# gorgonia/agogo

Hardware: AMD Instinct MI355X
Metric: mcts_sims_per_sec (higher is better)
Workload: dtype f32 (Winograd F(5x5,3x3): fp32 transforms; transform-domain products as fp16x2 = each fp32 operand scaled by a power of two and split into 2 fp16 pieces (22-23 significand bits, absolute error <= 2^-38 of the tensor range), 3 fp16 MFMAs per product, fp32 accumulate)

## Files before the change

### agogo_amd/capi.py

```python
import ctypes as C
import os

import numpy as np

_HERE = os.path.dirname(os.path.abspath(__file__))
_LIB = None

NONE, BLACK, WHITE = 0, 1, 2
PASS, RESIGN = -1, -2
NO_MOVE = -32768
GAME_MNK, GAME_C4, GAME_KOMI, GAME_WQ = 0, 1, 2, 3
ENC_TWOPLANE, ENC_WQ = 0, 1
INF_NET, INF_DUMMY, INF_SCRIPT, INF_HASH, INF_UNIFORM, INF_CALLBACK = 0, 1, 2, 3, 4, 5
BN_DEGENERATE_EPS, BN_RUNNING, BN_IDENTITY = 0, 1, 2
COMPUTE_F32_MFMA, COMPUTE_BF16X3, COMPUTE_FP16X2, COMPUTE_WINO, COMPUTE_AUTO, COMPUTE_WINO_H2 = 0, 1, 2, 3, 4, 5
COMPUTE_FORCE = 0x100
PROF_CONV, PROF_HEADS, PROF_SELECT, PROF_EXPAND, PROF_MOVE, PROF_CONV_INIT = 0, 1, 2, 3, 4, 5
PROF_WINO_IN, PROF_WINO_GEMM, PROF_WINO_OUT = 6, 7, 8
DONT_PREFER_PASS, PREFER_PASS, DONT_RESIGN = 0, 1, 2
POOL_STRICT, POOL_STOP_SEARCH, POOL_GROW = 0, 1, 2


class AgzError(RuntimeError):
    pass
# ... 113 lines not shown
    sig("agz_net_set_bn_stats", i32, vp, i32, pf, pf, C.c_size_t)
    sig("agz_net_init_random", i32, vp, u64)
    sig("agz_net_commit", i32, vp)
    sig("agz_net_infer", i32, vp, pf, i32, pf, pf)
    sig("agz_net_infer_dev", i32, vp, vp, i32, vp, vp)
    sig("agz_host_alloc", i32, vp, C.c_size_t, pvp)
    sig("agz_host_free", i32, vp, vp)
    sig("agz_mcts_to_dot", i32, vp, i32, C.c_char_p, C.c_size_t, C.POINTER(C.c_size_t))
    sig("agz_mcts_set_timeout_ms", i32, vp, i32)
    sig("agz_mcts_last_simulations", i32, vp, C.POINTER(C.c_int64))
    sig("agz_net_set_latency_mode", i32, vp, i32)
    sig("agz_net_set_tower_queues", i32, vp, i32)
    sig("agz_net_set_compute_mode", i32, vp, i32)
    sig("agz_net_flops_per_eval", f64, vp)
    sig("agz_net_save", i32, vp, C.c_char_p)
    sig("agz_net_load", i32, vp, C.c_char_p)
    sig("agz_arena_get_results", i32, vp, C.POINTER(C.c_int64), C.POINTER(C.c_int64), C.POINTER(C.c_int64))
    sig("agz_trainer_create", i32, vp, C.POINTER(NetConf), pvp)
    sig("agz_trainer_destroy", None, vp)
    sig("agz_trainer_num_params", i32, vp)
    sig("agz_trainer_param_info", i32, vp, i32, C.c_char_p, C.c_size_t, C.POINTER(C.c_size_t))
    sig("agz_trainer_set_param", i32, vp, i32, pf, C.c_size_t)
    sig("agz_trainer_get_param", i32, vp, i32, pf, C.c_size_t)
    sig("agz_trainer_get_grad", i32, vp, i32, pf, C.c_size_t)
    sig("agz_trainer_init_random", i32, vp, u64)
    sig("agz_trainer_batch", i32, vp, pf, pf, pf, C.c_float, pf)
    sig("agz_trainer_forward_backward", i32, vp, pf, pf, pf, pf)
    sig("agz_trainer_forward_backward_dev", i32, vp, vp, vp, vp, pf)
    sig("agz_trainer_apply", i32, vp, C.c_float, C.c_float)
    sig("agz_trainer_grads_dev", i32, vp, pvp, C.POINTER(C.c_size_t))
    sig("agz_trainer_set_solver", i32, vp, C.POINTER(SolverConf))
    sig("agz_trainer_get_solver", i32, vp, C.POINTER(SolverConf))
    sig("agz_trainer_get_velocity", i32, vp, i32, pf, C.c_size_t)
    sig("agz_trainer_set_velocity", i32, vp, i32, pf, C.c_size_t)
    sig("agz_trainer_reset_solver", i32, vp)
    sig("agz_trainer_set_compute_mode", i32, vp, i32)
    sig("agz_train", i32, vp, pf, pf, pf, i32, i32, u64, pf)
    sig("agz_trainer_export", i32, vp, vp)
    sig("agz_trainer_save", i32, vp, C.c_char_p)
    sig("agz_trainer_load", i32, vp, C.c_char_p)
    sig("agz_arena_create", i32, vp, C.POINTER(GameConf), C.POINTER(MctsConf), i32, u64, i32, pvp)
    sig("agz_arena_destroy", None, vp)
    sig("agz_arena_set_inferencer", i32, vp, i32, i32, vp)
    sig("agz_arena_reset", i32, vp, pu8)
    sig("agz_arena_play", i32, vp, i32, i32)
    sig("agz_arena_selfplay", i32, vp, C.c_int64, i32)
    sig("agz_arena_set_parallel", i32, vp, i32)
    sig("agz_arena_begin_move", i32, vp)
    sig("agz_arena_simulate", i32, vp, i32)
    sig("agz_arena_end_move", i32, vp, i32)
    sig("agz_arena_apply_moves", i32, vp, pi)
    sig("agz_arena_get_stats", i32, vp, C.POINTER(ArenaStats))
    sig("agz_arena_get_game", i32, vp, i32, pi, C.POINTER(GameState))
    sig("agz_arena_get_history", i32, vp, i32, pi, i32, pi)
    sig("agz_arena_root_children", i32, vp, i32, i32, pi, pu, pf, pf, i32, pi)
    sig("agz_arena_tree_nodes", i32, vp, i32, i32, pi)
    sig("agz_arena_get_examples", i32, vp, pf, pf, pf, pi, i32, pi)
    sig("agz_arena_clear_examples", i32, vp)
    sig("agz_arena_drop_labelled_examples", i32, vp)
    sig("agz_arena_examples_dev", i32, vp, pvp, pvp, pvp, pi)
    i64, pi64 = C.c_int64, C.POINTER(C.c_int64)
    sig("agz_train_dev", i32, vp, vp, vp, vp, i32, i32, u64, pf)
    sig("agz_examples_create", i32, vp, i32, i32, i32, i32, pvp)
    sig("agz_examples_destroy", None, vp)
    sig("agz_examples_count", i32, vp, pi64)
    sig("agz_examples_clear", i32, vp)
    sig("agz_examples_append_arena", i32, vp, vp)
    sig("agz_examples_append_dev", i32, vp, vp, vp, vp, i64)
    sig("agz_examples_append_host", i32, vp, pf, pf, pf, i64)
    sig("agz_examples_get", i32, vp, pf, pf, pf, i64, pi64)
    sig("agz_examples_augment_rotate", i32, vp)
    sig("agz_examples_prepare", i32, vp, i32, i32, u64, pi)
    sig("agz_examples_tensors_dev", i32, vp, pvp, pvp, pvp, pi64, pi)
    sig("agz_examples_get_tensors", i32, vp, pf, pf, pf)
    sig("agz_examples_raw_dev", i32, vp, pvp, pvp, pvp)
    sig("agz_rotate_boards", i32, vp, pf, i32, i32, i32, pf)
    sig("agz_ctx_prof_set_stride", i32, vp, i32, i32)
    sig("agz_wino_stages", i32, vp, pf, pf, i32, i32, i32, i32, i32, pf, pf)
    sig("agz_wino_h2_tile", i32, i32, i32)
    sig("agz_net_set_wino_h2_form", i32, vp, i32)
    sig("agz_net_set_wino_h2_gemm", i32, vp, i32)
    sig("agz_net_min_same_batch", i32, vp, i32, i32, C.POINTER(C.c_int))
    sig("agz_arena_set_prep_compact", i32, vp, i32)
    sig("agz_trainer_set_dma_forward", i32, vp, i32)
    sig("agz_arena_last_prep_batch", i32, vp, C.POINTER(C.c_int), C.POINTER(C.c_int))
    sig("agz_arena_debug_counter", i32, vp, i32, C.POINTER(C.c_int64))
    sig("agz_arena_pool_capacity", i32, vp, C.POINTER(C.c_int), C.POINTER(C.c_int))
    sig("agz_wino_h2_chained", i32, i32, i32, i32)
    sig("agz_arena_random_moves", i32, vp, pi, u64)
    sig("agz_arena_set_state", i32, vp, i32, C.POINTER(State))
    sig("agz_arena_examples_labelled_dev", i32, vp, pvp)
    sig("agz_mcts_create", i32, vp, C.POINTER(GameConf), C.POINTER(MctsConf), u64, i32, pvp)
    sig("agz_mcts_destroy", None, vp)
    sig("agz_mcts_set_inferencer", i32, vp, i32, vp)
    sig("agz_mcts_set_inferencer_callback", i32, vp, INFER_FN, vp, i32)
    sig("agz_arena_set_inferencer_callback", i32, vp, i32, INFER_FN, vp, i32)
    sig("agz_arena_set_pool_policy", i32, vp, i32)
    sig("agz_mcts_set_pool_policy", i32, vp, i32)
    sig("agz_mcts_set_parallel", i32, vp, i32)
    sig("agz_mcts_set_game", i32, vp, C.POINTER(State))
    sig("agz_mcts_search", i32, vp, i32, pi)
    sig("agz_mcts_policies", i32, vp, pf, i32)
    sig("agz_mcts_root_children", i32, vp, pi, pu, pf, pf, i32, pi)
    sig("agz_mcts_nodes", i32, vp, pi)
    sig("agz_mcts_children", i32, vp, i32, pi, pi, pu, pf, pf, i32, pi)
    sig("agz_mcts_get_stats", i32, vp, C.POINTER(ArenaStats))
    sig("agz_mcts_reset", i32, vp)
    sig("agz_comm_init_all", i32, pvp, i32, pvp)
    sig("agz_comm_unique_id", i32, vp)
    sig("agz_comm_init_rank", i32, vp, i32, i32, vp, pvp)
    sig("agz_comm_destroy", None, vp)
    sig("agz_comm_rank", i32, vp)
    sig("agz_comm_size", i32, vp)
    sig("agz_examples_allgather", i32, vp, vp)
    sig("agz_trainer_allreduce", i32, vp, vp)
    sig("agz_trainer_forward_backward_allreduce", i32, vp, vp, pf, pf, pf, pf)
    sig("agz_trainer_forward_backward_allreduce_dev", i32, vp, vp, vp, vp, vp, pf)
    sig("agz_comm_debug_fail_slice", i32, vp, i32)
    sig("agz_trainer_create_sharded", i32, vp, C.POINTER(NetConf), pvp)
    sig("agz_trainer_shard", i32, vp, C.POINTER(i32), C.POINTER(i32), C.POINTER(i32))
    sig("agz_comm_debug_fail_layer", i32, vp, i32)
    _LIB = L
    return L


def _check(r, what=""):
    if r != 0:
        raise AgzError("%s failed (%d): %s" % (what, r, lib().agz_last_error().decode(errors="replace")))


def _pf(a):
    return a.ctypes.data_as(C.POINTER(C.c_float))


def _pi(a):
    return a.ctypes.data_as(C.POINTER(C.c_int32))


class Ctx:
    def __init__(self, device=0):
        self.h = C.c_void_p()
        self._children = []
        _check(lib().agz_ctx_create(device, C.byref(self.h)), "agz_ctx_create")

    def _adopt(self, child):
        import weakref
        self._children.append(weakref.ref(child))

    def close(self):
        if self.h:
            kids = [r() for r in self._children]
            for k in sorted([k for k in kids if k is not None], key=lambda k: 0 if isinstance(k, Arena) else 1):
                k.close()
            self._children = []
            for p in list(getattr(self, "_pinned", {}).values()):
                lib().agz_host_free(self.h, C.c_void_p(p))
            self._pinned = {}
            lib().agz_ctx_destroy(self.h)
            self.h = C.c_void_p()

    def __del__(self):
        try:
            self.close()
        except Exception:
            pass

# ... 314 lines not shown
        self._nets.append(cfn)

    def set_pool_policy(self, policy):
        _check(lib().agz_arena_set_pool_policy(self.h, int(policy)), "agz_arena_set_pool_policy")

    def reset(self, a_is_black=None):
        if a_is_black is None:
            _check(lib().agz_arena_reset(self.h, None), "agz_arena_reset")
        else:
            a = np.ascontiguousarray(a_is_black, dtype=np.uint8)
            assert a.size == self.n_games
            _check(lib().agz_arena_reset(self.h, a.ctypes.data_as(C.POINTER(C.c_uint8))), "agz_arena_reset")

    def play(self, n_moves=0, record=True):
        _check(lib().agz_arena_play(self.h, n_moves, int(record)), "agz_arena_play")

    def selfplay(self, n_games_target, record=True):
        _check(lib().agz_arena_selfplay(self.h, n_games_target, int(record)), "agz_arena_selfplay")

    def set_parallel(self, lanes):
        _check(lib().agz_arena_set_parallel(self.h, int(lanes)), "agz_arena_set_parallel")

    def begin_move(self):
        _check(lib().agz_arena_begin_move(self.h), "agz_arena_begin_move")

    def simulate(self, k):
        _check(lib().agz_arena_simulate(self.h, k), "agz_arena_simulate")

    def end_move(self, record=True):
        _check(lib().agz_arena_end_move(self.h, int(record)), "agz_arena_end_move")

    def apply_moves(self, moves):
        m = np.ascontiguousarray(moves, dtype=np.int32)
        assert m.size == self.n_games
        _check(lib().agz_arena_apply_moves(self.h, _pi(m)), "agz_arena_apply_moves")

    def stats(self):
        s = ArenaStats()
        _check(lib().agz_arena_get_stats(self.h, C.byref(s)), "agz_arena_get_stats")
        return {f: getattr(s, f) for f, _ in ArenaStats._fields_}

    def random_moves(self, n_moves, seed=1337):
        m = np.ascontiguousarray(n_moves, dtype=np.int32)
        assert m.size == self.n_games
        _check(lib().agz_arena_random_moves(self.h, _pi(m), seed), "agz_arena_random_moves")

    def set_state(self, g, **kw):
        st, keep = make_state(self.m * self.n, **kw)
        _check(lib().agz_arena_set_state(self.h, g, C.byref(st)), "agz_arena_set_state")
        del keep

    def results(self):
        a, b, d = C.c_int64(0), C.c_int64(0), C.c_int64(0)
        _check(lib().agz_arena_get_results(self.h, C.byref(a), C.byref(b), C.byref(d)), "agz_arena_get_results")
        return {"a_wins": a.value, "b_wins": b.value, "draws": d.value}

    def game(self, g):
        board = np.zeros(self.m * self.n, dtype=np.int32)
        st = GameState()
        _check(lib().agz_arena_get_game(self.h, g, _pi(board), C.byref(st)), "agz_arena_get_game")
        return board, {f: getattr(st, f) for f, _ in GameState._fields_ if f != "reserved"}

    def history(self, g):
        a = np.zeros(4096, dtype=np.int32)
        n = C.c_int32(0)
        _check(lib().agz_arena_get_history(self.h, g, _pi(a), a.size, C.byref(n)), "agz_arena_get_history")
        return a[:n.value].copy()

    def root_children(self, g, agent):
        cap = self.m * self.n + 2
        mv = np.zeros(cap, dtype=np.int32)
        vis = np.zeros(cap, dtype=np.uint32)
        bs = np.zeros(cap, dtype=np.float32)
        pr = np.zeros(cap, dtype=np.float32)
        n = C.c_int32(0)
        _check(lib().agz_arena_root_children(self.h, g, agent, _pi(mv), vis.ctypes.data_as(C.POINTER(C.c_uint32)),
                                             _pf(bs), _pf(pr), cap, C.byref(n)), "agz_arena_root_children")
        k = n.value
        return mv[:k].copy(), vis[:k].copy(), bs[:k].copy(), pr[:k].copy()

    def set_prep_compact(self, on=True):
        _check(lib().agz_arena_set_prep_compact(self.h, int(on)), "agz_arena_set_prep_compact")

    def last_prep_batch(self):
        b, r = C.c_int(0), C.c_int(0)
        _check(lib().agz_arena_last_prep_batch(self.h, C.byref(b), C.byref(r)), "agz_arena_last_prep_batch")
        return b.value, r.value

    def pool_capacity(self):
        c, g = C.c_int(0), C.c_int(0)
        _check(lib().agz_arena_pool_capacity(self.h, C.byref(c), C.byref(g)), "agz_arena_pool_capacity")
        return c.value, g.value

    def max_path_nodes(self):
        v = C.c_int64(0)
        _check(lib().agz_arena_debug_counter(self.h, 15, C.byref(v)), "agz_arena_debug_counter")
        return v.value

    def tree_nodes(self, g, agent):
        n = C.c_int32(0)
        _check(lib().agz_arena_tree_nodes(self.h, g, agent, C.byref(n)), "agz_arena_tree_nodes")
        return n.value

    def examples(self):
        n = C.c_int32(0)
        _check(lib().agz_arena_get_examples(self.h, None, None, None, None, 0, C.byref(n)), "agz_arena_get_examples")
        k = n.value
        cells = self.m * self.n
        planes = np.zeros((k, self.features * cells), np.float32)
        policy = np.zeros((k, self.action_space + 1), np.float32)
        value = np.zeros(k, np.float32)
        gidx = np.zeros(k, np.int32)
        if k:
            _check(lib().agz_arena_get_examples(self.h, _pf(planes), _pf(policy), _pf(value), _pi(gidx), k,
                                                C.byref(n)), "agz_arena_get_examples")
        return planes, policy, value, gidx

    def clear_examples(self):
        _check(lib().agz_arena_clear_examples(self.h), "agz_arena_clear_examples")


def make_state(cells, board, to_move, n_moves=0, passes=0, hash=0, captures=(0.0, 0.0), last_moves=(), historical=()):
    b = np.ascontiguousarray(board, dtype=np.int32).reshape(-1)
    assert b.size == cells
    lm = np.ascontiguousarray(last_moves, dtype=np.int32).reshape(-1)
    hs = np.ascontiguousarray(historical, dtype=np.int32).reshape(-1)
    assert hs.size % cells == 0
    st = State()
    st.board = _pi(b)
    st.to_move, st.n_moves, st.passes, st.hash = int(to_move), int(n_moves), int(passes), int(hash) & 0xFFFFFFFF
    st.captures_black, st.captures_white = float(captures[0]), float(captures[1])
    st.last_moves = _pi(lm) if lm.size else None
    st.n_last_moves = lm.size
    st.historical = _pi(hs) if hs.size else None
    st.n_historical = hs.size // cells
    return st, [b, lm, hs]


class Mcts:

    def __init__(self, ctx, kind, m, n, k=0, komi=0.0, encoder=ENC_TWOPLANE, seed=1337, max_nodes=0, max_moves=0, PUCT=1.0,
                 M=None, N=None, RandomCount=0, Budget=100, RandomMinVisits=0, RandomTemperature=0.0, DumbPass=True,
                 ResignPercentage=0.0, PassPreference=DONT_PREFER_PASS):
        self.ctx = ctx
        self.kind, self.m, self.n = kind, m, n
        self.action_space = n if kind == GAME_C4 else m * n
        self.gconf = GameConf(kind, m, n, k, komi, max_moves, encoder)
        self.mconf = MctsConf(PUCT, M if M is not None else m, N if N is not None else n, RandomCount, Budget,
                              RandomMinVisits, RandomTemperature, int(DumbPass), ResignPercentage, PassPreference)
        self.h = C.c_void_p()
        self._nets = []
        _check(lib().agz_mcts_create(ctx.h, C.byref(self.gconf), C.byref(self.mconf), seed, max_nodes, C.byref(self.h)),
               "agz_mcts_create")
        ctx._adopt(self)

    def close(self):
        if self.h and self.ctx.h:
            lib().agz_mcts_destroy(self.h)
        self.h = C.c_void_p()

    def __del__(self):
        try:
            self.close()
        except Exception:
            pass

# ... 265 lines not shown
```

### agogo_amd/csrc/common.hpp

```cpp
#pragma once
#include <hip/hip_runtime.h>

#include <cstdarg>
#include <cstdint>
#include <cstdio>
#include <string>
#include <vector>

#include "../../include/agz_debug.h"

namespace agz {

void set_error(const char* fmt, ...);
const char* get_error();

#define AGZ_HIP_TRY(expr)                                                                      \
  do {                                                                                         \
    hipError_t _e = (expr);                                                                    \
    if (_e != hipSuccess) {                                                                    \
      agz::set_error("%s:%d: %s -> %s", __FILE__, __LINE__, #expr, hipGetErrorString(_e));     \
      return AGZ_E_HIP;                                                                        \
    }                                                                                          \
  } while (0)

#define AGZ_REQUIRE(cond, code, ...)  \
  do {                                \
    if (!(cond)) {                    \
      agz::set_error(__VA_ARGS__);    \
      return (code);                  \
    }                                 \
  } while (0)

struct ProfClass {
  std::vector<std::pair<hipEvent_t, hipEvent_t>> pairs;
  size_t used = 0;
  int64_t launches = 0;
  double total_ms = 0;
};

}

struct agz_ctx {
  int device = 0;
  hipStream_t stream = nullptr;
  hipStream_t stream2 = nullptr;
  hipEvent_t ev_fork = nullptr, ev_join = nullptr;
  bool prof_on = false;
  unsigned prof_mask = ~0u;
  int prof_stride[AGZ_PROF_NCLASS];
  int64_t prof_seen[AGZ_PROF_NCLASS] = {};
  agz_ctx() { for (auto& v : prof_stride) v = 1; }
  agz::ProfClass prof[AGZ_PROF_NCLASS];
  int prof_open = 0;
  int num_cus = 256;
  unsigned func_attr_state = 0;

  void prof_begin(int klass);
  void prof_end(int klass);
  int prof_collect();
};

namespace agz {
struct ProfScope {
  agz_ctx* c;
  int k;
  bool on;
  ProfScope(agz_ctx* c_, int k_) : c(c_), k(k_), on(c_->prof_on && ((c_->prof_mask >> k_) & 1u) && (c_->prof_seen[k_]++ % c_->prof_stride[k_]) == 0) { if (on) c->prof_begin(k); }
  ~ProfScope() { if (on) c->prof_end(k); }
};

struct ProfScopeOn {
  agz_ctx* c;
  int k;
  bool on;
  ProfScopeOn(agz_ctx* c_, int k_, bool enable)
      : c(c_), k(k_), on(enable && c_->prof_on && ((c_->prof_mask >> k_) & 1u) && (c_->prof_seen[k_]++ % c_->prof_stride[k_]) == 0) { if (on) c->prof_begin(k); }
  ~ProfScopeOn() { if (on) c->prof_end(k); }
};

inline int ceil_div(int a, int b) { return (a + b - 1) / b; }
inline int round_up(int a, int b) { return ceil_div(a, b) * b; }

struct SplitMix64 {
  uint64_t s;
  explicit SplitMix64(uint64_t seed = 0) : s(seed) {}
  uint64_t next() {
    uint64_t z = (s += 0x9E3779B97F4A7C15ull);
    z = (z ^ (z >> 30)) * 0xBF58476D1CE4E5B9ull;
    z = (z ^ (z >> 27)) * 0x94D049BB133111EBull;
    return z ^ (z >> 31);
  }
  int32_t int31() { return (int32_t)(next() >> 33); }
  double float64() { return (double)(next() >> 11) * (1.0 / 9007199254740992.0); }
};
}
```

### agogo_amd/csrc/conv_wino_h2.hpp

```cpp
#pragma once

template <int TM> struct WinoT;
template <> struct WinoT<4> {
  static constexpr int AL = 6, VSHIFT = 7;
  static constexpr float BT[6][6] = {{4, 0, -5, 0, 1, 0}, {0, -4, -4, 1, 1, 0}, {0, 4, -4, -1, 1, 0}, {0, -2, -1, 2, 1, 0}, {0, 2, -1, -2, 1, 0}, {0, 4, 0, -5, 0, 1}};
  static constexpr float AT[4][6] = {{1, 1, 1, 1, 1, 0}, {0, 1, -1, 2, -2, 0}, {0, 1, 1, 4, 4, 0}, {0, 1, -1, 8, -8, 1}};
  static constexpr double G[6][3] = {{1.0 / 4, 0, 0}, {-1.0 / 6, -1.0 / 6, -1.0 / 6}, {-1.0 / 6, 1.0 / 6, -1.0 / 6}, {1.0 / 24, 1.0 / 12, 1.0 / 6}, {1.0 / 24, -1.0 / 12, 1.0 / 6}, {0, 0, 1}};
};
template <> struct WinoT<5> {
  static constexpr int AL = 7, VSHIFT = 6;
  static constexpr float BT[7][7] = {{-0.5f, 0.25f, 2.5f, -1.25f, -2, 1, 0}, {0, 0.5f, 0.25f, -2.25f, -1, 1, 0}, {0, -0.5f, 0.75f, 1.75f, -3, 1, 0},
                                     {0, 1, 1.5f, -2, -1.5f, 1, 0},          {0, -1, 2.5f, 0, -2.5f, 1, 0},       {0, 0.25f, 0, -1.25f, 0, 1, 0},
                                     {0, -0.5f, 0.25f, 2.5f, -1.25f, -2, 1}};
  static constexpr float AT[5][7] = {{1, 1, 1, 1, 1, 1, 0}, {0, 1, -1, 0.5f, -0.5f, 2, 0}, {0, 1, 1, 0.25f, 0.25f, 4, 0}, {0, 1, -1, 0.125f, -0.125f, 8, 0},
                                     {0, 1, 1, 0.0625f, 0.0625f, 16, 1}};
  static constexpr double G[7][3] = {{-2, 0, 0}, {-2.0 / 3, -2.0 / 3, -2.0 / 3}, {-2.0 / 9, 2.0 / 9, -2.0 / 9}, {16.0 / 9, 8.0 / 9, 4.0 / 9}, {16.0 / 15, -8.0 / 15, 4.0 / 15},
                                     {2.0 / 45, 4.0 / 45, 8.0 / 45}, {0, 0, 1}};
};
template <int TM> __device__ __forceinline__ void wino_btv(const float* d, float* o);
template <int TM> __device__ __forceinline__ void wino_atv(const float* m, float* o);
template <> __device__ __forceinline__ void wino_btv<4>(const float* d, float* o) { wino_bt6(d, o); }
template <> __device__ __forceinline__ void wino_atv<4>(const float* m, float* o) { wino_at4(m, o); }
template <> __device__ __forceinline__ void wino_btv<5>(const float* d, float* o) {
  o[0] = -0.5f * d[0] + 0.25f * d[1] + 2.5f * d[2] - 1.25f * d[3] - 2.f * d[4] + d[5];
// ... 992 lines not shown
static void wino_build_u2(std::vector<_Float16>& u2, int Ntot, int C, Get get, std::vector<float>& t_in, std::vector<float>& col_unscale) {
  using WT = WinoT<TM>;
  constexpr int AL = WT::AL, NP = AL * AL;
  const int NC = C / 32;
  std::vector<float> U((size_t)NP * Ntot * C, 0.f);
  std::vector<float> rmax(C, 0.f);
  for (int n = 0; n < Ntot; n++)
    for (int ci = 0; ci < C; ci++) {
      double g[3][3], tg[AL][3];
      bool any = false;
      for (int i = 0; i < 3; i++) for (int j = 0; j < 3; j++) { g[i][j] = get(n, ci, i * 3 + j); any = any || g[i][j] != 0.0; }
      if (!any) continue;
      for (int xi = 0; xi < AL; xi++) for (int j = 0; j < 3; j++) tg[xi][j] = WT::G[xi][0] * g[0][j] + WT::G[xi][1] * g[1][j] + WT::G[xi][2] * g[2][j];
      for (int xi = 0; xi < AL; xi++) for (int nu = 0; nu < AL; nu++) {
        const float v = (float)(tg[xi][0] * WT::G[nu][0] + tg[xi][1] * WT::G[nu][1] + tg[xi][2] * WT::G[nu][2]);
        U[((size_t)(xi * AL + nu) * Ntot + n) * C + ci] = v;
        rmax[ci] = std::max(rmax[ci], std::fabs(v));
      }
    }
  t_in.assign(C, 1.0f);
  for (int ci = 0; ci < C; ci++)
    if (rmax[ci] > 0.f && std::isfinite(rmax[ci])) {
      int ex = 0;
      std::frexp(rmax[ci], &ex);
      ex = std::max(-100, std::min(100, ex - 1));
      t_in[ci] = std::ldexp(1.0f, ex);
    }
  std::vector<float> cmax(Ntot, 0.f);
  for (int pos = 0; pos < NP; pos++)
    for (int n = 0; n < Ntot; n++)
      for (int ci = 0; ci < C; ci++) {
        float& v = U[((size_t)pos * Ntot + n) * C + ci];
        v /= t_in[ci];
        cmax[n] = std::max(cmax[n], std::fabs(v));
      }
  col_unscale.assign(Ntot, 1.0f);
  std::vector<float> su(Ntot, 1.0f);
  for (int n = 0; n < Ntot; n++)
    if (cmax[n] > 0.f && std::isfinite(cmax[n])) {
      int ex = 0;
      std::frexp(cmax[n], &ex);
      su[n] = std::ldexp(1.0f, 14 - ex);
      col_unscale[n] = 1.0f / su[n];
    }
  u2.assign((size_t)NP * NC * 2 * Ntot * 32, (_Float16)0.f);
  for (int pos = 0; pos < NP; pos++)
    for (int n = 0; n < Ntot; n++)
      for (int ci = 0; ci < C; ci++) {
        const float xs = U[((size_t)pos * Ntot + n) * C + ci] * su[n];
        const _Float16 hi = (_Float16)xs;
        const _Float16 lo = (_Float16)(xs - (float)hi);
        const size_t base = ((((size_t)pos * NC + ci / 32) * 2) * Ntot + n) * 32 + (ci % 32);
        u2[base] = hi;
        u2[base + (size_t)Ntot * 32] = lo;
      }
}

static inline int wino_h2_pick_tm(int H, int W) {
  static const int force = [] { const char* e = getenv("AGZ_WINO_H2_TM"); return e ? atoi(e) : 0; }();
  if (force == 4 || force == 5) return force;
  const int r4 = 36 * ceil_div(H, 4) * ceil_div(W, 4), r5 = 49 * ceil_div(H, 5) * ceil_div(W, 5);
  return r5 < r4 ? 5 : 4;
}

static inline size_t wino_h2_rows(int npos, size_t tiles, int row_pad = 0) { return (size_t)npos * (((tiles + 127) / 128) * (size_t)(128 + row_pad)); }

static void wino_h2_launch(agz_ctx* ctx, WinoH2Args& h, bool wide, hipStream_t st = nullptr) {
  if (!st) st = ctx->stream;
  WinoArgs& a = h.w;
  const int tm = h.tm == 5 ? 5 : 4;
  h.tm = tm; h.npos = (tm + 2) * (tm + 2);
  a.nty = ceil_div(a.H, tm); a.ntx = ceil_div(a.W, tm); a.TPB = a.nty * a.ntx; a.T = a.B * a.TPB;
  h.rsh = 7; h.rmask = 127; h.rB = 128u + (unsigned)h.row_pad; h.rA = (unsigned)h.npos * h.rB;
  a.n_mtiles = ceil_div(a.T, 128); a.n_ntiles = ceil_div(a.Ntot, 128);
  h.in_swap = a.C % 128 == 0 ? 1 : 0;
  const bool fits32 = (size_t)h.npos * h.rB * a.Ntot * 4 < ((size_t)1 << 32);
  int form = tm == 5 ? 3 : 0;
  if (form == 3 && !fits32) form = 0;
  const bool fuse = a.C % 128 == 0 && h.wave_max != nullptr;
  h.wm_per_board = a.TPB * (a.Cout_p >> 6);
  h.fuse_prev = (h.fuse_prev && fuse) ? 1 : 0;
  h.amax_self = const_cast<unsigned*>(h.amax_in);
  {
    ProfScopeOn ps(ctx, AGZ_PROF_WINO_IN, st == ctx->stream);
    const size_t n_in = (size_t)a.T * (a.C / 2);
    if (tm == 5) hipLaunchKernelGGL(wino_in_h2_kernel<5>, dim3((unsigned)((n_in + 255) / 256)), dim3(256), 0, st, h);
    else hipLaunchKernelGGL(wino_in_h2_kernel<4>, dim3((unsigned)((n_in + 255) / 256)), dim3(256), 0, st, h);
  }
  {
    ProfScopeOn ps(ctx, AGZ_PROF_WINO_GEMM, st == ctx->stream);
    const dim3 gw(h.npos * a.n_mtiles * ceil_div(a.Ntot, 256)), gn(h.npos * a.n_mtiles * a.n_ntiles);
    const int nk = a.C >> 5;
    bool done = true;
#define AGZ_H2D(NK_, PF_, NT_, G_) hipLaunchKernelGGL((wino_gemm_h2d_kernel<NK_, PF_, NT_>), G_, dim3(256), 0, st, h)
#define AGZ_H2D_NK(NK_) { if (wide) AGZ_H2D(NK_, 2, 2, gw); else AGZ_H2D(NK_, 2, 1, gn); }
    if (a.C & 31) done = false;
    else if (nk == 8) AGZ_H2D_NK(8)
    else if (nk == 2) AGZ_H2D_NK(2)
    else if (nk == 4) AGZ_H2D_NK(4)
    else if (nk == 6) AGZ_H2D_NK(6)
    else if (nk == 12) AGZ_H2D_NK(12)
    else if (nk == 16) AGZ_H2D_NK(16)
    else done = false;
#undef AGZ_H2D_NK
#undef AGZ_H2D
    if (done) {}
    else if (wide) hipLaunchKernelGGL(wino_gemm_h2w_kernel, gw, dim3(256), 0, st, h);
    else hipLaunchKernelGGL(wino_gemm_h2_kernel, gn, dim3(256), 0, st, h);
  }
  {
    ProfScopeOn ps(ctx, AGZ_PROF_WINO_OUT, st == ctx->stream);
    const size_t n_out = (size_t)a.T * a.Cout_p;
    if (h.raw) {
      const unsigned bd = a.Ntot % 256 == 0 ? 256u : (a.Ntot % 128 == 0 ? 128u : (a.Ntot % 64 == 0 ? 64u : 32u));
      const dim3 gr((unsigned)a.T, (unsigned)a.Ntot / bd);
      if (tm == 5) hipLaunchKernelGGL(wino_out_raw_h2_kernel<5>, gr, dim3(bd), 0, st, h);
      else hipLaunchKernelGGL(wino_out_raw_h2_kernel<4>, gr, dim3(bd), 0, st, h);
    } else if (form == 3 && (a.Cout_p % 256 == 0 || a.Cout_p == 128)) {
      const dim3 gq((unsigned)a.T, (unsigned)ceil_div(a.Cout_p, 256));
      if (tm == 5) hipLaunchKernelGGL(wino_out_quad_h2_kernel<5>, gq, dim3(7 * 64), 0, st, h);
      else hipLaunchKernelGGL(wino_out_quad_h2_kernel<4>, gq, dim3(6 * 64), 0, st, h);
    } else if (form == 3) {
      const unsigned bd = a.Cout_p % 256 == 0 ? 256u : (a.Cout_p % 128 == 0 ? 128u : 64u);
      const dim3 gs((unsigned)a.T, (unsigned)a.Cout_p / bd);
      if (tm == 5) hipLaunchKernelGGL(wino_out_seq_h2_kernel<5>, gs, dim3(bd), 0, st, h);
      else hipLaunchKernelGGL(wino_out_seq_h2_kernel<4>, gs, dim3(bd), 0, st, h);
    } else {
      if (tm == 5) hipLaunchKernelGGL(wino_out_h2_kernel<5>, dim3((unsigned)((n_out + 255) / 256)), dim3(256), 0, st, h);
      else hipLaunchKernelGGL(wino_out_h2_kernel<4>, dim3((unsigned)((n_out + 255) / 256)), dim3(256), 0, st, h);
    }
    if (h.wave_max && h.amax_out && !fuse)
      hipLaunchKernelGGL(wino_board_max_kernel, dim3(a.B), dim3(64), 0, st, h.wave_max, h.amax_out, h.wm_per_board);
  }
}
```

### agogo_amd/csrc/conv_wino_h2c.hpp

```cpp
#pragma once

__device__ __forceinline__ unsigned h2c_img(int row, int slot) { return maps::h2c_img(row, slot); }

template <int NK, int PFA>
__global__ __launch_bounds__(256, 2) void wino_gemm_h2c_kernel(WinoH2Args h) {
  const WinoArgs& a = h.w;
  constexpr int SA = 128 * 128, SB = 256 * 128;
  __shared__ __attribute__((aligned(16))) unsigned char lds[SA + SB];

  const int n_nt = a.Ntot >> 8;
  const int per_pos = a.n_mtiles * n_nt;
  const int nblk = h.npos * per_pos;
  const int id = blockIdx.x;
  int q = nblk >> 3, rr = nblk & 7, xcd = id & 7, slot = id >> 3;
  int tile = (xcd < rr ? xcd * (q + 1) : rr * (q + 1) + (xcd - rr) * q) + slot;
  const int pos = tile / per_pos;
  const int rem = tile - pos * per_pos;
  const int m_tile = rem / n_nt, n_tile = rem - m_tile * n_nt;

  const int tid = threadIdx.x, lane = tid & 63, wid = tid >> 6;
  const int wm = wid >> 1, wn = wid & 1;
  const unsigned st_lds = h2c_img(tid >> 3, tid & 7);
  const char* abase = reinterpret_cast<const char*>(a.V) + ((size_t)m_tile * h.npos + pos) * (size_t)NK * SA + (size_t)tid * 16;
  const char* bbase = reinterpret_cast<const char*>(h.U2c) + (((size_t)pos * NK) * n_nt + n_tile) * (size_t)SB + (size_t)tid * 16;
// ... 696 lines not shown
        for (int xi = 0; xi < AL; xi++) m[nu][xi] = h2_ldf4<MAUX>(mr, m_lane, m_soff(g2, s2, xi * AL + nu));
    }
    __builtin_amdgcn_sched_barrier(0);
    const unsigned v_base = (unsigned)((((g >> 3) * h.npos) * NS + s)) * 16384u + (unsigned)(g & 7) * 2048u;
    const unsigned v_pos = (unsigned)NS * 16384u;
    const float* yr = ybase;
    asm volatile("" : "+v"(yr));
#pragma unroll
    for (int i0 = 0; i0 < AL; i0 += 3) {
      constexpr int NRMAX = 3;
      const int nr = AL - i0 < NRMAX ? AL - i0 : NRMAX;
      f2c tmr[NRMAX][AL];
#pragma unroll
      for (int j = 0; j < AL; j++) {
        f2c d[AL];
#pragma unroll
        for (int ii = 0; ii < AL; ii++) {
          const float2 v = *reinterpret_cast<const float2*>(yr + (ii * PW + j) * 32);
          d[ii] = f2c{v.x, v.y};
        }
#pragma unroll
        for (int r = 0; r < NRMAX; r++)
          if (r < nr) tmr[r][j] = wino_bt_row_p<TM>(i0 + r, d);
      }
      __builtin_amdgcn_sched_barrier(0);
#pragma unroll
      for (int r = 0; r < NRMAX; r++) {
        if (r >= nr) continue;
        const int i = i0 + r;
        f2c o[AL];
        wino_btv_p<TM>(tmr[r], o);
#pragma unroll
        for (int j = 0; j < AL; j++) {
          unsigned lo;
          const unsigned hi = wino_h2_pack(o[j].x * sv, o[j].y * sv, &lo);
          const auto s16 = __builtin_amdgcn_permlane16_swap(hi, lo, false, false);
          const unsigned e0 = s16[0], e1 = s16[1];
          const auto s32 = __builtin_amdgcn_permlane32_swap(e0, e1, false, false);
          const unsigned w0 = s32[0], w1 = s32[1];
          __builtin_amdgcn_raw_buffer_store_b32(w0, vr, v_lane, v_base + (unsigned)(i * AL + j) * v_pos, VAUX);
          __builtin_amdgcn_raw_buffer_store_b32(w1, vr, v_lane + 256u, v_base + (unsigned)(i * AL + j) * v_pos, VAUX);
        }
      }
      __builtin_amdgcn_sched_barrier(0);
    }
    __syncthreads();
  }
}

static void wino_build_u2c(const std::vector<_Float16>& u2, std::vector<_Float16>& u2c, int npos, int Ntot, int C, int Cout_p) {
  const int NC = C / 32, NT = Ntot / 256;
  u2c.assign(u2.size(), (_Float16)0.f);
  for (int pos = 0; pos < npos; pos++)
    for (int kc = 0; kc < NC; kc++)
      for (int nn = 0; nn < Ntot; nn++) {
        const int s = nn >> 6, j2 = nn & 63, ch = 32 * s + (j2 >> 1), br = j2 & 1, n = br * Cout_p + ch;
        for (int p = 0; p < 2; p++) {
          const _Float16* src = &u2[((((size_t)pos * NC + kc) * 2 + p) * Ntot + n) * 32];
          _Float16* dst = &u2c[((((size_t)pos * NC + kc) * NT + (nn >> 8)) * 256 + (nn & 255)) * 64 + p * 32];
          for (int k = 0; k < 32; k++) dst[k] = src[k];
        }
      }
}

static inline bool wino_h2c_ok(int H, int W, int tm, int Kp) {
  const int tpb = ceil_div(H, tm) * ceil_div(W, tm);
  const int nk = Kp / 32;
  return Kp % 128 == 0 && 16 % tpb == 0 && (nk == 4 || nk == 8 || nk == 12 || nk == 16) &&
         (size_t)(16 / tpb) * (tm * ceil_div(H, tm) + 2) * (tm * ceil_div(W, tm) + 2) * 128 <= 80 * 1024;
}

static void wino_h2c_geometry(WinoH2Args& h) {
  WinoArgs& a = h.w;
  const int tm = h.tm == 5 ? 5 : 4;
  h.tm = tm; h.npos = (tm + 2) * (tm + 2);
  a.nty = ceil_div(a.H, tm); a.ntx = ceil_div(a.W, tm); a.TPB = a.nty * a.ntx; a.T = a.B * a.TPB;
  h.rsh = 7; h.rmask = 127; h.rA = (unsigned)h.npos * 128u; h.rB = 128u;
  a.n_mtiles = ceil_div(a.T, 128); a.n_ntiles = ceil_div(a.Ntot, 128);
  h.in_swap = 1; h.cform = 1; h.wm_per_board = 0;
}
static void wino_h2c_in(agz_ctx* ctx, WinoH2Args& h, hipStream_t st) {
  wino_h2c_geometry(h);
  h.fuse_prev = 0; h.amax_self = const_cast<unsigned*>(h.amax_in);
  ProfScopeOn ps(ctx, AGZ_PROF_WINO_IN, st == ctx->stream);
  const size_t n_in = (size_t)h.w.T * (h.w.C / 2);
  if (h.tm == 5) hipLaunchKernelGGL(wino_in_h2_kernel<5>, dim3((unsigned)((n_in + 255) / 256)), dim3(256), 0, st, h);
  else hipLaunchKernelGGL(wino_in_h2_kernel<4>, dim3((unsigned)((n_in + 255) / 256)), dim3(256), 0, st, h);
}
constexpr int WINO_H2_GEMM_DEFAULT = 1;
static void wino_h2c_gemm(agz_ctx* ctx, WinoH2Args& h, hipStream_t st) {
  wino_h2c_geometry(h);
  ProfScopeOn ps(ctx, AGZ_PROF_WINO_GEMM, st == ctx->stream);
  const dim3 g(h.npos * h.w.n_mtiles * (h.w.Ntot >> 8));
  const bool dma_ok = wino_h2_rows(h.npos, (size_t)h.w.T) * h.w.C * 4 < ((size_t)1 << 31) && (size_t)h.npos * h.w.C * h.w.Ntot * 4 < ((size_t)1 << 31);
  const int variant_all = h.gemm_variant > 0 ? h.gemm_variant : WINO_H2_GEMM_DEFAULT;
  const int variant = variant_all & 15, mode = (variant_all >> 4) & 3;
  const int n_slabs = h.w.Ntot >> 7;
  if (variant == 2 && dma_ok && (h.w.C >> 5) == 8 && h.w.Ntot % 256 == 0 && ctx->num_cus / 8 >= n_slabs) {
    const dim3 gp((unsigned)(8 * ((ctx->num_cus / 8) / n_slabs) * n_slabs));
    switch (mode) {
      case 1: hipLaunchKernelGGL(wino_gemm_h2p_kernel<1>, gp, dim3(256), 0, st, h); break;
      case 2: hipLaunchKernelGGL(wino_gemm_h2p_kernel<2>, gp, dim3(256), 0, st, h); break;
      case 3: hipLaunchKernelGGL(wino_gemm_h2p_kernel<3>, gp, dim3(256), 0, st, h); break;
      default: hipLaunchKernelGGL(wino_gemm_h2p_kernel<0>, gp, dim3(256), 0, st, h); break;
    }
    return;
  }
  if (dma_ok && h.temporal_stores && (h.w.C >> 5) == 8) { hipLaunchKernelGGL((wino_gemm_h2g_kernel<8, false>), g, dim3(256), 0, st, h); return; }
  if (dma_ok) {
    switch (h.w.C >> 5) {
      case 4: hipLaunchKernelGGL((wino_gemm_h2g_kernel<4>), g, dim3(256), 0, st, h); return;
      case 8: hipLaunchKernelGGL((wino_gemm_h2g_kernel<8>), g, dim3(256), 0, st, h); return;
      case 12: hipLaunchKernelGGL((wino_gemm_h2g_kernel<12>), g, dim3(256), 0, st, h); return;
      default: hipLaunchKernelGGL((wino_gemm_h2g_kernel<16>), g, dim3(256), 0, st, h); return;
    }
  }
  switch (h.w.C >> 5) {
    case 4: hipLaunchKernelGGL((wino_gemm_h2c_kernel<4, 2>), g, dim3(256), 0, st, h); break;
    case 8: hipLaunchKernelGGL((wino_gemm_h2c_kernel<8, 2>), g, dim3(256), 0, st, h); break;
    case 12: hipLaunchKernelGGL((wino_gemm_h2c_kernel<12, 2>), g, dim3(256), 0, st, h); break;
    default: hipLaunchKernelGGL((wino_gemm_h2c_kernel<16, 2>), g, dim3(256), 0, st, h); break;
  }
}
static void wino_h2c_oi(agz_ctx* ctx, WinoH2Args& h, bool last, hipStream_t st, int variant = 4) {
  wino_h2c_geometry(h);
  ProfScopeOn ps(ctx, AGZ_PROF_WINO_OUT, st == ctx->stream);
  const WinoArgs& a = h.w;
  const dim3 g((unsigned)ceil_div(a.T, 16), (unsigned)(a.C >> 5));
  const size_t shm = last ? 0 : (size_t)(16 / a.TPB) * a.H * a.W * 32 * sizeof(float);
  const bool fits31 = wino_h2_rows(h.npos, (size_t)a.T) * a.Ntot * 4 < ((size_t)1 << 31);
  if (variant == 4 && !last && fits31 && !(ctx->func_attr_state & 2u)) {
    const bool ok = hipFuncSetAttribute(reinterpret_cast<const void*>(&wino_oip_h2c_kernel<5>), hipFuncAttributeMaxDynamicSharedMemorySize, 80 * 1024) == hipSuccess &&
                    hipFuncSetAttribute(reinterpret_cast<const void*>(&wino_oip_h2c_kernel<4>), hipFuncAttributeMaxDynamicSharedMemorySize, 80 * 1024) == hipSuccess;
    if (!ok) (void)hipGetLastError();
    ctx->func_attr_state |= 2u | (ok ? 1u : 0u);
  }
  if (variant == 4 && !last && fits31 && (ctx->func_attr_state & 1u)) {
    const size_t shp = (size_t)(16 / a.TPB) * (h.tm * a.nty + 2) * (h.tm * a.ntx + 2) * 32 * sizeof(float);
    const int items = ceil_div(a.T, 16) * (a.C >> 5);
    const dim3 gp((unsigned)std::min(items, 2 * ctx->num_cus));
    if (h.tm == 5 && h.temporal_stores) {
      (void)hipFuncSetAttribute(reinterpret_cast<const void*>(&wino_oip_h2c_kernel<5, false>), hipFuncAttributeMaxDynamicSharedMemorySize, 80 * 1024);
      hipLaunchKernelGGL((wino_oip_h2c_kernel<5, false>), gp, dim3(256), shp, st, h);
      return;
    }
    if (h.tm == 5) hipLaunchKernelGGL((wino_oip_h2c_kernel<5>), gp, dim3(256), shp, st, h);
    else hipLaunchKernelGGL((wino_oip_h2c_kernel<4>), gp, dim3(256), shp, st, h);
    return;
  }
  if (h.tm == 5) {
    if (last) hipLaunchKernelGGL((wino_oi_h2c_kernel<5, true>), g, dim3(256), shm, st, h);
    else hipLaunchKernelGGL((wino_oi_h2c_kernel<5, false>), g, dim3(256), shm, st, h);
  } else {
    if (last) hipLaunchKernelGGL((wino_oi_h2c_kernel<4, true>), g, dim3(256), shm, st, h);
    else hipLaunchKernelGGL((wino_oi_h2c_kernel<4, false>), g, dim3(256), shm, st, h);
  }
}
```

### agogo_amd/csrc/ctx.hip

```cpp
#include "common.hpp"

namespace agz {
static thread_local char g_err[1024] = "";
void set_error(const char* fmt, ...) {
  va_list ap;
  va_start(ap, fmt);
  vsnprintf(g_err, sizeof(g_err), fmt, ap);
  va_end(ap);
}
const char* get_error() { return g_err; }
}

void agz_ctx::prof_begin(int klass) {
  agz::ProfClass& p = prof[klass];
  if (p.used == p.pairs.size()) {
    hipEvent_t a, b;
    if (hipEventCreate(&a) != hipSuccess || hipEventCreate(&b) != hipSuccess) return;
    p.pairs.push_back({a, b});
  }
  hipEventRecord(p.pairs[p.used].first, stream);
  prof_open++;
}
void agz_ctx::prof_end(int klass) {
  agz::ProfClass& p = prof[klass];
  if (p.used >= p.pairs.size()) return;
  hipEventRecord(p.pairs[p.used].second, stream);
  p.used++;
  if (prof_open > 0) prof_open--;
  if (p.used >= 4096 && prof_open == 0) prof_collect();
}
int agz_ctx::prof_collect() {
  AGZ_HIP_TRY(hipStreamSynchronize(stream));
  for (int k = 0; k < AGZ_PROF_NCLASS; k++) {
    agz::ProfClass& p = prof[k];
    for (size_t i = 0; i < p.used; i++) {
      float ms = 0;
      if (hipEventElapsedTime(&ms, p.pairs[i].first, p.pairs[i].second) == hipSuccess) {
        p.total_ms += ms;
        p.launches++;
      }
    }
    p.used = 0;
  }
  return AGZ_OK;
}

extern "C" {

const char* agz_last_error(void) { return agz::get_error(); }
const char* agz_version(void) { return "libagz 0.1 (gfx950, HIP, fp32 MFMA conv tower, device MCTS)"; }

int agz_ctx_create(int device, agz_ctx** out) {
  AGZ_REQUIRE(out != nullptr, AGZ_E_INVALID, "agz_ctx_create: out is NULL");
  int n = 0;
  hipError_t e = hipGetDeviceCount(&n);
  if (e != hipSuccess || n <= 0) {
    agz::set_error("agz_ctx_create: no HIP device available (%s) — libagz has no CPU fallback",
                   e == hipSuccess ? "device count 0" : hipGetErrorString(e));
    return AGZ_E_HIP;
  }
  AGZ_REQUIRE(device >= 0 && device < n, AGZ_E_INVALID, "agz_ctx_create: device %d out of range [0,%d)", device, n);
  AGZ_HIP_TRY(hipSetDevice(device));
  agz_ctx* c = new agz_ctx();
  c->device = device;
  hipDeviceProp_t prop;
  AGZ_HIP_TRY(hipGetDeviceProperties(&prop, device));
  c->num_cus = prop.multiProcessorCount;
  AGZ_HIP_TRY(hipStreamCreateWithFlags(&c->stream, hipStreamNonBlocking));
  *out = c;
  return AGZ_OK;
}
int agz_host_alloc(agz_ctx* ctx, size_t bytes, void** out) {
  AGZ_REQUIRE(ctx && out && bytes > 0, AGZ_E_INVALID, "agz_host_alloc: bad argument");
  AGZ_HIP_TRY(hipSetDevice(ctx->device));
  void* p = nullptr;
  hipError_t e = hipHostMalloc(&p, bytes, hipHostMallocDefault);
  if (e != hipSuccess) { agz::set_error("agz_host_alloc: %zu bytes of pinned host memory: %s", bytes, hipGetErrorString(e)); return AGZ_E_NOMEM; }
  *out = p;
  return AGZ_OK;
}

int agz_host_free(agz_ctx* ctx, void* p) {
  AGZ_REQUIRE(ctx, AGZ_E_INVALID, "agz_host_free: ctx is NULL");
  if (!p) return AGZ_OK;
  AGZ_HIP_TRY(hipSetDevice(ctx->device));
  AGZ_HIP_TRY(hipHostFree(p));
  return AGZ_OK;
}

void agz_ctx_destroy(agz_ctx* c) {
  if (!c) return;
  hipSetDevice(c->device);
  hipStreamSynchronize(c->stream);
  for (auto& p : c->prof)
    for (auto& pr : p.pairs) { hipEventDestroy(pr.first); hipEventDestroy(pr.second); }
  if (c->stream2) hipStreamDestroy(c->stream2);
  if (c->ev_fork) hipEventDestroy(c->ev_fork);
  if (c->ev_join) hipEventDestroy(c->ev_join);
  hipStreamDestroy(c->stream);
  delete c;
}
int agz_ctx_sync(agz_ctx* c) {
  AGZ_REQUIRE(c, AGZ_E_INVALID, "ctx is NULL");
  AGZ_HIP_TRY(hipStreamSynchronize(c->stream));
  return AGZ_OK;
}
void* agz_ctx_stream(agz_ctx* c) { return c ? (void*)c->stream : nullptr; }
int agz_ctx_prof_enable(agz_ctx* c, int enable) {
  AGZ_REQUIRE(c, AGZ_E_INVALID, "ctx is NULL");
  if (enable) {
    AGZ_HIP_TRY(hipStreamSynchronize(c->stream));
    for (auto& p : c->prof) { p.used = 0; p.launches = 0; p.total_ms = 0; }
    c->prof_mask = enable == 1 ? ~0u : ((unsigned)enable >> 1);
    c->prof_on = true;
  } else {
    c->prof_on = false;
    return c->prof_collect();
  }
  return AGZ_OK;
}
int agz_ctx_prof_set_stride(agz_ctx* c, int klass, int stride) {
  AGZ_REQUIRE(c && klass >= 0 && klass < AGZ_PROF_NCLASS && stride >= 1, AGZ_E_INVALID, "agz_ctx_prof_set_stride: bad argument");
  c->prof_stride[klass] = stride;
  c->prof_seen[klass] = 0;
  return AGZ_OK;
}
int agz_ctx_prof_read(agz_ctx* c, int klass, int64_t* launches, double* total_ms) {
  AGZ_REQUIRE(c && klass >= 0 && klass < AGZ_PROF_NCLASS, AGZ_E_INVALID, "bad prof class");
  int r = c->prof_collect();
  if (r != AGZ_OK) return r;
  if (launches) *launches = c->prof[klass].launches;
  if (total_ms) *total_ms = c->prof[klass].total_ms;
  return AGZ_OK;
}

}
```

### agogo_amd/csrc/engine.hip

```cpp
#include <algorithm>
#include <chrono>
#include <climits>
#include <cstring>
#include <vector>

#include "engine_dev.hpp"
#include "net.hpp"

namespace agz {

__device__ __forceinline__ size_t pool_base(const Dev& d, int t, int pool) { return ((size_t)t * 2 + pool) * d.cap; }

__device__ __forceinline__ float evaluate(float bs, uint32_t visits, int player) {
  float score = __fdiv_rn(bs, (float)visits);
  if (player == AGZ_WHITE) score = __fsub_rn(1.0f, score);
  return score;
}

__device__ __forceinline__ float sqrt_cr(float x) {
  if (!(x > 0.f)) return x == 0.f ? x : __builtin_amdgcn_sqrtf(x);
  float r = __builtin_amdgcn_sqrtf(x);
  while ((double)r * (double)r > (double)x) r = __uint_as_float(__float_as_uint(r) - 1u);
  float rn = __uint_as_float(__float_as_uint(r) + 1u);
  while ((double)rn * (double)rn <= (double)x) { r = rn; rn = __uint_as_float(__float_as_uint(r) + 1u); }
// ... 277 lines not shown
  if (lane == 0) { d.stalled[t] = 0; d.overflow[t] = 0; }
  int pool = d.cur_pool[t];
  size_t base = pool_base(d, t, pool);
  bool ok = d.has_root[t] && d.has_prev[t] && c.kind != AGZ_GAME_C4;
  int depth = 0, node = 0;
  if (ok) {
    int prev_ply = d.prev_ply[t];
    depth = st.ply - prev_ply;
    if (depth < 0 || prev_ply < d.hist_from[g]) ok = false;
    if (ok && c.kind != AGZ_GAME_WQ) {
      int bad = 0;
      for (int i = lane; i < c.cells; i += WAVE) {
        int v = s.board[i];
        for (int k = 0; k < depth; k++) { int mv = d.moves[(size_t)g * d.moves_stride + st.ply - 1 - k]; if (mv == i) v = AGZ_NONE; }
        if (v != d.prev_board[(size_t)t * CELLS_PAD + i]) bad = 1;
      }
      if (__syncthreads_or(bad)) ok = false;
    }
    for (int k = 0; ok && k < depth; k++) {
      int mv = d.moves[(size_t)g * d.moves_stride + prev_ply + k];
      int off = d.kids_off[base + node], n = off >= 0 ? d.kids_n[base + node] : 0;
      int found = 0x7fffffff;
      for (int i = lane; i < n; i += WAVE) if (d.nmove[base + off + i] == mv && i < found) found = i;
      for (int o = 32; o > 0; o >>= 1) { int f2 = __shfl_xor(found, o, 64); found = f2 < found ? f2 : found; }
      if (found == 0x7fffffff) ok = false; else node = off + found;
    }
  }
  if (ok) {
    if (node != 0) {
      size_t nb = pool_base(d, t, pool ^ 1);
      if (lane == 0) {
        d.prior[nb] = d.prior[base + node]; d.visits[nb] = d.visits[base + node]; d.bsum[nb] = d.bsum[base + node];
        d.kids_off[nb] = d.kids_off[base + node]; d.kids_n[nb] = d.kids_n[base + node]; d.nmove[nb] = d.nmove[base + node];
      }
      __syncthreads();
      int new_n = 1, scan = 0;
      while (scan < new_n) {
        int hi = min(scan + WAVE, new_n);
        int i = scan + lane;
        int ooff = (i < hi) ? d.kids_off[nb + i] : -1;
        unsigned long long m = __ballot(ooff >= 0);
        while (m) {
          int src_lane = __ffsll((long long)m) - 1;
          m &= m - 1;
          int so = __shfl(ooff, src_lane, 64);
          int ni = scan + src_lane;
          int cnt = d.kids_n[nb + ni];
          for (int k = lane; k < cnt; k += WAVE) {
            d.prior[nb + new_n + k] = d.prior[base + so + k];
            d.visits[nb + new_n + k] = d.visits[base + so + k];
            d.bsum[nb + new_n + k] = d.bsum[base + so + k];
            d.kids_off[nb + new_n + k] = d.kids_off[base + so + k];
            d.kids_n[nb + new_n + k] = d.kids_n[base + so + k];
            d.nmove[nb + new_n + k] = d.nmove[base + so + k];
          }
          if (lane == 0) d.kids_off[nb + ni] = new_n;
          new_n += cnt;
        }
        __syncthreads();
        scan = hi;
      }
      if (lane == 0) { d.cur_pool[t] = pool ^ 1; d.n_nodes[t] = new_n; }
    }
  } else {
    int rootmv = AGZ_PASS;
    if (!c.pass_legal) {
      if (c.go_like) analyse(c, s, nullptr, lane, false);
      int first = 0x7fffffff;
      for (int i = lane; i < c.A; i += WAVE) {
        bool legal = c.go_like ? go_legal(c, s, i, player) : (s.board[i] == AGZ_NONE);
        if (legal && i < first) first = i;
      }
      for (int o = 32; o > 0; o >>= 1) { int f2 = __shfl_xor(first, o, 64); first = f2 < first ? f2 : first; }
      rootmv = first == 0x7fffffff ? AGZ_PASS : first;
    }
    if (lane == 0) {
      d.prior[base] = 0.f; d.visits[base] = 1; d.bsum[base] = 0.f; d.kids_off[base] = -1; d.kids_n[base] = 0;
      d.nmove[base] = (int16_t)rootmv; d.n_nodes[t] = 1; d.has_root[t] = 1;
    }
  }
  if (lane == 0) d.has_prev[t] = 0;
}

__global__ __launch_bounds__(64) void k_select(Dev d, GameCfg c, MctsCfg mc, float* act_in0, float* act_in1, int prep, int nl) {
  __shared__ Sh s;
  int g = blockIdx.x, lane = threadIdx.x;
  const size_t q0 = (size_t)g * d.V;
  if (d.ended[g]) { if (lane < nl) d.leaf_kind[q0 + lane] = LEAF_NONE; return; }
  int agent = agent_of(d, g);
  int t = agent * d.G + g;
  if (d.stalled[t]) { if (lane < nl) { d.leaf_kind[q0 + lane] = LEAF_NULL; d.path_len[q0 + lane] = 0; } return; }
  const bool use_ring = c.encoder == AGZ_ENC_WQ;
  const bool use_vl = d.V > 1;
  size_t base = pool_base(d, t, d.cur_pool[t]);
  for (int l = 0; l < nl; l++) {
    const size_t q = q0 + l;
    if (l > 0) { __threadfence(); __syncthreads(); }
    St st;
    load_state(c, d, g, s, st, use_ring, lane);
    int32_t* path = d.path + q * MAXPATH;
    int node = 0, depth = 1, plen = 1, kind = LEAF_NONE;
    int kids_seen = 0;
    float result = 0.f;
    if (lane == 0) path[0] = 0;
    while (true) {
      if (depth > mc.maxDepth) { kind = LEAF_NULL; plen--; break; }
      if (use_vl && lane == 0) d.vl[base + node] = 1;
      int off = d.kids_off[base + node];
      if (off < 0) {
        if (c.has_passes && st.passes >= 2) {
          if (prep) { kind = LEAF_TERMINAL; result = 0.f; }
          else {
            analyse(c, s, nullptr, lane);
            float b, w;
            area_scores(c, s, lane, &b, &w);
            result = __fsub_rn(__fsub_rn(b, w), c.komi);
            kind = LEAF_TERMINAL;
          }
        } else {
          kind = LEAF_EXPAND;
        }
        break;
      }
      if (prep) { kind = LEAF_NONE; break; }
      int n = d.kids_n[base + node];
      kids_seen += n;
      int mv;
      int ci = select_child(d, base, off, n, st.to_move, mc.PUCT, lane, use_vl, &mv);
      if (ci < 0) { kind = LEAF_NULL; break; }
      int child = off + ci;
      apply_move(c, d, s, st, mv, use_ring, lane);
      if (lane == 0) path[plen] = child;
      plen++;
      node = child;
      depth++;
    }
    if (kind == LEAF_EXPAND) {
      if (c.go_like) analyse(c, s, nullptr, lane, false);
      legal_mask(c, s, st.to_move, d.leaf_legal + q * CELLS_PAD, lane);
      for (int i = lane; i < c.cells; i += WAVE) d.leaf_board[q * CELLS_PAD + i] = s.board[i];
      float* act = agent == 0 ? act_in0 : act_in1;
      if (act) encode_nhwc(c, s, st, act + ((size_t)l * d.G + d.slot_of_game[g]) * (c.m + 2) * (c.n + 2) * 32, lane);
      if (d.cb_planes && ((d.cb_mask >> agent) & 1)) encode_nchw(c, s, st, d.cb_planes + q * (size_t)c.F * c.cells, lane);
    }
    if (lane == 0) {
      d.leaf_kind[q] = kind;
      d.leaf_player[q] = st.to_move;
      d.leaf_ply[q] = move_number(c, st.ply);
      d.leaf_result[q] = result;
      d.path_len[q] = plen;
      if (prep && kind == LEAF_EXPAND) atomicAdd(&d.counters[CNT_PREP_EXPAND], 1ull);
      if (!prep) {
        atomicAdd(&d.counters[CNT_PATH], (unsigned long long)plen);
        atomicAdd(&d.counters[CNT_KIDS], (unsigned long long)kids_seen);
        atomicMax(&d.counters[CNT_PATHMAX], (unsigned long long)plen);
      }
    }
    __syncthreads();
  }
}

__global__ __launch_bounds__(64) void k_select_paths(Dev d, GameCfg c, MctsCfg mc, int prep, int nl) {
  const int g = blockIdx.x, lane = threadIdx.x;
  const size_t q0 = (size_t)g * d.V;
  if (d.ended[g]) { if (lane < nl) d.leaf_kind[q0 + lane] = LEAF_NONE; return; }
  const int agent = agent_of(d, g);
  const int t = agent * d.G + g;
  if (d.stalled[t]) { if (lane < nl) { d.leaf_kind[q0 + lane] = LEAF_NULL; d.path_len[q0 + lane] = 0; } return; }
  const size_t base = pool_base(d, t, d.cur_pool[t]);
// ... 151 lines not shown
  {
    int rnk[RANK_PER];
    stable_desc_ranks(s.fscore, n, lane, rnk);
#pragma unroll
    for (int k = 0; k < RANK_PER; k++) {
      const int i = lane + k * WAVE;
      if (i < n) { d.exp_score[q * CELLS_PAD + rnk[k]] = s.fscore[i]; d.exp_move[q * CELLS_PAD + rnk[k]] = (int16_t)s.fmove[i]; }
    }
  }
  if (lane == 0) { d.exp_n[q] = n; d.exp_value[q] = value; }
}

__global__ __launch_bounds__(64) void k_expand_commit(Dev d, GameCfg c, MctsCfg mc, int prep, int nl) {
  const int g = blockIdx.x, lane = threadIdx.x;
  if (d.ended[g]) return;
  const int agent = agent_of(d, g);
  const int t = agent * d.G + g;
  const size_t q0 = (size_t)g * d.V;
  const size_t base = pool_base(d, t, d.cur_pool[t]);
  int n_null = 0, n_lanes = 0;
  unsigned have_mask = 0;
  for (int l = 0; l < nl; l++) {
    const size_t q = q0 + l;
    if (l > 0) { __threadfence(); __syncthreads(); }
    const int kind = d.leaf_kind[q];
    if (kind == LEAF_NONE) continue;
    n_lanes++;
    if (!prep && lane == 0) atomicAdd(&d.counters[CNT_SIMS], 1ull);
    const int32_t* path = d.path + q * MAXPATH;
    const int plen = d.path_len[q];
    if (kind == LEAF_NULL) {
      n_null++;
      for (int j = lane; j < plen; j += WAVE) d.vl[base + path[j]] = 0;
      continue;
    }
    const int node = path[plen - 1];
    float result = d.leaf_result[q];
    bool have = true, follower = false;
    if (kind == LEAF_EXPAND && l > 0) {
      for (int l2 = 0; l2 < l && !follower; l2++) {
        const size_t q2 = q0 + l2;
        if (d.leaf_kind[q2] == LEAF_EXPAND && d.path_len[q2] == plen && d.path[q2 * MAXPATH + plen - 1] == node) {
          follower = true;
          result = d.leaf_result[q2];
          have = (have_mask >> l2) & 1u;
        }
      }
    }
    if (kind == LEAF_EXPAND && !follower) {
      const int n = d.exp_n[q];
      result = d.exp_value[q];
      if (n > 0) {
        const int off = d.n_nodes[t];
        if (off + n > d.cap) {
          if (lane == 0) { if (!d.overflow[t]) atomicAdd(&d.counters[CNT_FULL], 1ull); d.overflow[t] = 1; d.stalled[t] = 1; }
          have = false;
        } else {
          for (int i = lane; i < n; i += WAVE) {
            const size_t o = base + off + i;
            d.prior[o] = d.exp_score[q * CELLS_PAD + i]; d.visits[o] = 1; d.bsum[o] = 0.f; d.kids_off[o] = -1; d.kids_n[o] = 0;
            d.nmove[o] = d.exp_move[q * CELLS_PAD + i];
          }
          if (lane == 0) { d.kids_off[base + node] = off; d.kids_n[base + node] = (int16_t)n; d.n_nodes[t] = off + n; }
        }
      }
      if (lane == 0) atomicAdd(&d.counters[CNT_EVALS], 1ull);
    }
    __syncthreads();
    if (lane == 0) d.leaf_result[q] = result;
    if (have) have_mask |= 1u << l;
    if (have) {
      for (int j = lane; j < plen; j += WAVE) {
        const size_t o = base + path[j];
        d.visits[o] = d.visits[o] + 1;
        d.bsum[o] = __fadd_rn(d.bsum[o], result);
      }
      if (!prep && lane == 0) atomicAdd(&d.counters[CNT_NONNULL], 1ull);
    }
    for (int j = lane; j < plen; j += WAVE) d.vl[base + path[j]] = 0;
  }
  if (n_lanes > 0 && n_null == n_lanes && lane == 0) d.stalled[t] = 1;
}

__global__ __launch_bounds__(64) void k_expand(Dev d, GameCfg c, MctsCfg mc, InfDesc inf, int prep, int nl) {
  __shared__ Sh s;
  int g = blockIdx.x, lane = threadIdx.x;
  if (d.ended[g]) return;
  int agent = agent_of(d, g);
  int t = agent * d.G + g;
  const size_t q0 = (size_t)g * d.V;
  const bool use_vl = d.V > 1;
  size_t base = pool_base(d, t, d.cur_pool[t]);
  int n_null = 0, n_lanes = 0;
  unsigned have_mask = 0;
  for (int l = 0; l < nl; l++) {
    const size_t q = q0 + l;
    if (l > 0) { __threadfence(); __syncthreads(); }
    int kind = d.leaf_kind[q];
    if (kind == LEAF_NONE) continue;
    n_lanes++;
    if (!prep && lane == 0) atomicAdd(&d.counters[CNT_SIMS], 1ull);
    const int32_t* path = d.path + q * MAXPATH;
    int plen = d.path_len[q];
    if (kind == LEAF_NULL) {
      n_null++;
      if (use_vl) for (int j = lane; j < plen; j += WAVE) d.vl[base + path[j]] = 0;
      continue;
    }
    int node = path[plen - 1];
    float result = d.leaf_result[q];
    bool have = true;
    bool follower = false;
    if (kind == LEAF_EXPAND && l > 0) {
      for (int l2 = 0; l2 < l && !follower; l2++) {
        const size_t q2 = q0 + l2;
        if (d.leaf_kind[q2] == LEAF_EXPAND && d.path_len[q2] == plen && d.path[q2 * MAXPATH + plen - 1] == node) {
          follower = true;
          result = d.leaf_result[q2];
          have = (have_mask >> l2) & 1u;
        }
      }
    }
    if (kind == LEAF_EXPAND && !follower) {
      int player = d.leaf_player[q];
      const uint8_t* legal = d.leaf_legal + q * CELLS_PAD;
      const int ik = inf.kind[agent];
      const int plen_pol = inf.policy_len[agent];
      const float* pol = nullptr;
      float value = 0.f;
      uint32_t ph = 0;
      if (ik == AGZ_INF_NET) {
        int slot = l * d.G + d.slot_of_game[g];
        pol = inf.policy[agent] + (size_t)slot * plen_pol;
        value = inf.value[agent][slot];
      } else if (ik == AGZ_INF_DUMMY) {
        int dp = inf.dummy_player[agent];
        value = dp == 1 ? 1.f : (dp == 2 ? -1.f : 0.f);
      } else if (ik == AGZ_INF_SCRIPT) {
        int mn = d.leaf_ply[q];
        value = (mn == 0 || mn == 1 || mn == 5) ? 0.5f : 0.f;
      } else if (ik == AGZ_INF_HASH) {
        uint32_t h = 0;
        for (int i = lane; i < c.cells; i += WAVE) h += mix32((uint32_t)i * 4u + (uint32_t)d.leaf_board[q * CELLS_PAD + i] + 1u);
        for (int o = 32; o > 0; o >>= 1) h += __shfl_xor(h, o, 64);
        h += mix32(0xABCD0000u + (uint32_t)player);
        ph = h;
        value = (float)(mix32(h ^ 0xDEADBEEFu) >> 8) * (1.0f / 16777216.0f);
      } else {
        value = 1 / 25.0f;
      }
      auto policy_at = [&](int i) -> float {
        switch (ik) {
          case AGZ_INF_NET: return pol[i];
          case AGZ_INF_DUMMY: return __fdiv_rn(1.f, (float)plen_pol);
          case AGZ_INF_SCRIPT: {
            int mn = d.leaf_ply[q];
            const int8_t cell[9] = {4, 0, 2, 6, 3, 5, 1, 7, 8};
            if (mn >= 0 && mn < 9 && i == cell[mn]) return (mn & 1) ? 0.1f : 0.9f;
            return 0.f;
          }
          case AGZ_INF_HASH: return (float)((mix32(ph + (uint32_t)i * 0x9E3779B9u) >> 8) + 1u) * (1.0f / 16777216.0f);
          default: return 1 / 25.0f;
        }
      };
      if (player == AGZ_WHITE) value = __fsub_rn(1.f, value);
      int n = 0;
      {
        constexpr int PER = CELLS_PAD / WAVE;
        uint8_t lg[PER]; float pr[PER];
// ... 383 lines not shown
      const bool ok = i < c.A && (c.go_like ? go_legal(c, s, i, player) : s.board[i] == AGZ_NONE);
      const unsigned long long m = __ballot(ok);
      const int cnt = __popcll(m);
      if (want >= seen && want < seen + cnt) {
        unsigned long long mm = m;
        for (int q = 0; q < want - seen; q++) mm &= mm - 1;
        mv = b0 + (__ffsll((long long)mm) - 1);
      }
      seen += cnt;
    }
  }
  if (lane == 0) { forced[g] = mv; remaining[g] = mv == AGZ_NO_MOVE ? 0 : remaining[g] - 1; }
}

}

using namespace agz;

struct agz_arena {
  agz_ctx* ctx = nullptr;
  GameCfg gc{};
  MctsCfg mc{};
  Dev d{};
  int G = 0;
  uint64_t seed = 0, seed0 = 0;
  std::vector<void*> allocs;
  int inf_kind[2] = {AGZ_INF_DUMMY, AGZ_INF_DUMMY};
  agz_net* net[2] = {nullptr, nullptr};
  float* d_policy[2] = {nullptr, nullptr};
  float* d_value[2] = {nullptr, nullptr};
  std::vector<uint8_t> a_is_black;
  int32_t* d_forced = nullptr;
  std::vector<int32_t> slot_host;
  int32_t* d_remaining = nullptr;
  unsigned long long prep_expand_seen = 0;
  bool prep_compact = true;
  int last_prep_batch = 0, last_prep_roots = 0;
  int nA_slots = 0, nB_slots = 0;
  bool in_move = false;
  bool restart = false;
  int moves_done = 0;
  agz_infer_fn cb_fn[2] = {nullptr, nullptr};
  void* cb_user[2] = {nullptr, nullptr};
  int cb_plen[2] = {0, 0};
  std::vector<void*> host_allocs;
  int cb_rows = 0;
  int32_t *h_kind = nullptr, *h_player = nullptr, *h_ply = nullptr, *h_tomove = nullptr, *h_ab = nullptr, *h_ended = nullptr;
  int8_t* h_lboard = nullptr;
  float* h_planes = nullptr;
  float *h_pk_planes = nullptr, *h_pk_policy = nullptr, *h_pk_value = nullptr;
  int32_t *h_pk_board = nullptr, *h_pk_tomove = nullptr, *h_pk_mn = nullptr, *h_pk_game = nullptr;
  float* h_policy[2] = {nullptr, nullptr};
  float* h_value[2] = {nullptr, nullptr};
  int64_t cb_calls = 0, cb_leaves = 0;
  bool pool_grow = false;
  long long room_sims = 0, sims_this_move = 0;
  int pool_grows = 0;
  int ensure_pool_room(long long sims);
  bool pool_stop = false;
  size_t h_pk_policy_cap = 0, h_policy_cap[2] = {0, 0}, h_value_cap[2] = {0, 0};

  template <typename T>
  int alloc(T** p, size_t n) {
    void* q = nullptr;
    AGZ_HIP_TRY(hipMalloc(&q, n * sizeof(T)));
    AGZ_HIP_TRY(hipMemsetAsync(q, 0, n * sizeof(T), ctx->stream));
    allocs.push_back(q);
    *p = (T*)q;
    return AGZ_OK;
  }
  bool split_nets() const { return inf_kind[0] == AGZ_INF_NET && inf_kind[1] == AGZ_INF_NET && net[0] != net[1]; }
  template <typename T>
  int halloc(T** p, size_t n) {
    void* q = nullptr;
    AGZ_HIP_TRY(hipHostMalloc(&q, std::max<size_t>(n, 1) * sizeof(T), hipHostMallocDefault));
    host_allocs.push_back(q);
    *p = (T*)q;
    return AGZ_OK;
  }
  int cb_setup();
  int cb_run(int nl);
  int update_slots();
  int nn_step(int prep, int nl = 1);
};

__global__ __launch_bounds__(256) void k_prep_compact(Dev d, float* act, int slot_f4) {
  const int i = blockIdx.x * 256 + threadIdx.x;
  float4* a4 = reinterpret_cast<float4*>(act);
  int rank = 0;
  for (int g = 0; g < d.G; g++) {
    const bool need = d.leaf_kind[(size_t)g * d.V] == LEAF_EXPAND && !d.ended[g];
    if (i == 0) d.prep_slot[g] = need ? rank : 0;
    if (!need) continue;
    const int src = d.slot_of_game[g];
    if (src != rank && i < slot_f4) a4[(size_t)rank * slot_f4 + i] = a4[(size_t)src * slot_f4 + i];
    rank++;
  }
}

__global__ __launch_bounds__(256) void k_pool_copy(Dev o, Dev n) {
  const int t = blockIdx.y;
  const int pool = o.cur_pool[t], cnt = o.n_nodes[t];
  const size_t so = ((size_t)t * 2 + pool) * o.cap, sn = ((size_t)t * 2 + pool) * n.cap;
  for (int i = blockIdx.x * 256 + threadIdx.x; i < cnt; i += gridDim.x * 256) {
    n.prior[sn + i] = o.prior[so + i]; n.visits[sn + i] = o.visits[so + i]; n.bsum[sn + i] = o.bsum[so + i];
    n.kids_off[sn + i] = o.kids_off[so + i]; n.kids_n[sn + i] = o.kids_n[so + i]; n.nmove[sn + i] = o.nmove[so + i];
  }
}

int agz_arena::ensure_pool_room(long long sims) {
  hipStream_t s = ctx->stream;
  const int T = d.T;
  std::vector<int32_t> nn(T);
  AGZ_HIP_TRY(hipMemcpyAsync(nn.data(), d.n_nodes, (size_t)T * 4, hipMemcpyDeviceToHost, s));
  AGZ_HIP_TRY(hipStreamSynchronize(s));
  long long most = 0;
  for (int t = 0; t < T; t++) most = std::max<long long>(most, nn[t]);
  const long long need = most + (sims + 2) * (long long)(gc.A + 1) + 16;
  if (need <= d.cap) return AGZ_OK;
  long long ncap = std::max(need + need / 2, 2ll * d.cap);
  size_t free_b = 0, total_b = 0;
  AGZ_HIP_TRY(hipMemGetInfo(&free_b, &total_b));
  const size_t per_node = 4 + 4 + 4 + 4 + 2 + 2 + 1;
  auto bytes = [&](long long c) { return (size_t)T * 2 * (size_t)c * per_node; };
  if (bytes(ncap) + (1ull << 30) > free_b) ncap = need;
  AGZ_REQUIRE(ncap < (1ll << 30) && bytes(ncap) + (256ull << 20) <= free_b, AGZ_E_NOMEM,
              "AGZ_POOL_GROW: the fullest tree holds %lld nodes, the next search may need %lld per pool — %zu MB for %d trees do not fit the free device memory (%zu MB)",
              most, need, bytes(need) >> 20, T, free_b >> 20);
  Dev nd = d;
  nd.cap = (int)ncap;
  const size_t pool = (size_t)T * 2 * (size_t)ncap;
  void* old[7] = {d.prior, d.visits, d.bsum, d.kids_off, d.kids_n, d.nmove, d.vl};
  int r;
  if ((r = alloc(&nd.prior, pool)) != AGZ_OK || (r = alloc(&nd.visits, pool)) != AGZ_OK || (r = alloc(&nd.bsum, pool)) != AGZ_OK ||
      (r = alloc(&nd.kids_off, pool)) != AGZ_OK || (r = alloc(&nd.kids_n, pool)) != AGZ_OK || (r = alloc(&nd.nmove, pool)) != AGZ_OK ||
      (r = alloc(&nd.vl, pool)) != AGZ_OK)
    return r;
  hipLaunchKernelGGL(k_pool_copy, dim3(64, T), dim3(256), 0, s, d, nd);
  AGZ_HIP_TRY(hipStreamSynchronize(s));
  for (void* p : old) {
    allocs.erase(std::remove(allocs.begin(), allocs.end(), p), allocs.end());
    hipFree(p);
  }
  d = nd;
  pool_grows++;
  return AGZ_OK;
}

int agz_arena::cb_setup() {
  const int rows = G * d.V;
  const size_t pl = (size_t)gc.F * gc.cells;
  if (!d.cb_planes || cb_rows != rows) {
    int r;
    if ((r = alloc(&d.cb_planes, (size_t)rows * pl)) != AGZ_OK) return r;
    if ((r = halloc(&h_kind, rows)) != AGZ_OK || (r = halloc(&h_player, rows)) != AGZ_OK || (r = halloc(&h_ply, rows)) != AGZ_OK ||
        (r = halloc(&h_tomove, G)) != AGZ_OK || (r = halloc(&h_ab, G)) != AGZ_OK || (r = halloc(&h_ended, G)) != AGZ_OK ||
        (r = halloc(&h_lboard, (size_t)rows * CELLS_PAD)) != AGZ_OK || (r = halloc(&h_planes, (size_t)rows * pl)) != AGZ_OK ||
        (r = halloc(&h_pk_planes, (size_t)rows * pl)) != AGZ_OK || (r = halloc(&h_pk_value, rows)) != AGZ_OK ||
        (r = halloc(&h_pk_board, (size_t)rows * gc.cells)) != AGZ_OK || (r = halloc(&h_pk_tomove, rows)) != AGZ_OK ||
        (r = halloc(&h_pk_mn, rows)) != AGZ_OK || (r = halloc(&h_pk_game, rows)) != AGZ_OK)
      return r;
    cb_rows = rows;
    h_pk_policy_cap = 0; h_policy_cap[0] = h_policy_cap[1] = 0; h_value_cap[0] = h_value_cap[1] = 0;
  }
  const size_t pk_need = (size_t)rows * std::max(std::max(cb_plen[0], cb_plen[1]), 1);
  if (pk_need > h_pk_policy_cap) { int r = halloc(&h_pk_policy, pk_need); if (r != AGZ_OK) return r; h_pk_policy_cap = pk_need; }
// ... 15 lines not shown
  return AGZ_OK;
}

int agz_arena::cb_run(int nl) {
  hipStream_t s = ctx->stream;
  const int rows = G * d.V;
  const size_t pl = (size_t)gc.F * gc.cells;
  AGZ_HIP_TRY(hipMemcpyAsync(h_kind, d.leaf_kind, (size_t)rows * 4, hipMemcpyDeviceToHost, s));
  AGZ_HIP_TRY(hipMemcpyAsync(h_player, d.leaf_player, (size_t)rows * 4, hipMemcpyDeviceToHost, s));
  AGZ_HIP_TRY(hipMemcpyAsync(h_ply, d.leaf_ply, (size_t)rows * 4, hipMemcpyDeviceToHost, s));
  AGZ_HIP_TRY(hipMemcpyAsync(h_tomove, d.to_move, (size_t)G * 4, hipMemcpyDeviceToHost, s));
  AGZ_HIP_TRY(hipMemcpyAsync(h_ab, d.a_is_black, (size_t)G * 4, hipMemcpyDeviceToHost, s));
  AGZ_HIP_TRY(hipMemcpyAsync(h_ended, d.ended, (size_t)G * 4, hipMemcpyDeviceToHost, s));
  AGZ_HIP_TRY(hipMemcpyAsync(h_lboard, d.leaf_board, (size_t)rows * CELLS_PAD, hipMemcpyDeviceToHost, s));
  AGZ_HIP_TRY(hipMemcpyAsync(h_planes, d.cb_planes, (size_t)rows * pl * 4, hipMemcpyDeviceToHost, s));
  AGZ_HIP_TRY(hipStreamSynchronize(s));
  for (int a = 0; a < 2; a++) {
    if (inf_kind[a] != AGZ_INF_CALLBACK) continue;
    if (a == 1 && inf_kind[0] == AGZ_INF_CALLBACK && cb_fn[0] == cb_fn[1] && cb_user[0] == cb_user[1] && cb_plen[0] == cb_plen[1]) continue;
    const bool both = a == 0 && inf_kind[1] == AGZ_INF_CALLBACK && cb_fn[0] == cb_fn[1] && cb_user[0] == cb_user[1] && cb_plen[0] == cb_plen[1];
    const int plen = cb_plen[a];
    int n = 0;
    std::vector<int> qs, ags;
    for (int g = 0; g < G; g++) {
      if (h_ended[g]) continue;
      const int agent = ((h_tomove[g] == AGZ_BLACK) == (h_ab[g] != 0)) ? 0 : 1;
      if (agent != a && !(both && agent == 1)) continue;
      for (int l = 0; l < nl; l++) {
        const int q = g * d.V + l;
        if (h_kind[q] != LEAF_EXPAND) continue;
        memcpy(h_pk_planes + (size_t)n * pl, h_planes + (size_t)q * pl, pl * sizeof(float));
        for (int i = 0; i < gc.cells; i++) h_pk_board[(size_t)n * gc.cells + i] = h_lboard[(size_t)q * CELLS_PAD + i];
        h_pk_tomove[n] = h_player[q]; h_pk_mn[n] = h_ply[q]; h_pk_game[n] = g;
        qs.push_back(q); ags.push_back(agent);
        n++;
      }
    }
    if (n == 0) continue;
    agz_leaf_batch b{};
    b.n = n; b.features = gc.F; b.height = gc.m; b.width = gc.n; b.policy_len = plen;
    b.planes = h_pk_planes; b.board = h_pk_board; b.to_move = h_pk_tomove; b.move_number = h_pk_mn; b.game = h_pk_game;
    b.policy = h_pk_policy; b.value = h_pk_value;
    memset(h_pk_policy, 0, (size_t)n * plen * sizeof(float));
    memset(h_pk_value, 0, (size_t)n * sizeof(float));
    const int rc = cb_fn[a](cb_user[a], &b);
    cb_calls++; cb_leaves += n;
    if (rc != 0) { agz::set_error("the host inferencer (AGZ_INF_CALLBACK, agent %d) returned %d for a batch of %d leaves: the search is aborted, reset the arena", a, rc, n); return AGZ_E_CALLBACK; }
    for (int i = 0; i < n; i++) {
      const int q = qs[i], g = q / d.V, l = q - g * d.V, ag = ags[i];
      const size_t slot = (size_t)l * G + slot_host[g];
      memcpy(h_policy[ag] + slot * plen, h_pk_policy + (size_t)i * plen, (size_t)plen * sizeof(float));
      h_value[ag][slot] = h_pk_value[i];
    }
  }
  for (int a = 0; a < 2; a++) {
    if (inf_kind[a] != AGZ_INF_CALLBACK) continue;
    AGZ_HIP_TRY(hipMemcpyAsync(d_policy[a], h_policy[a], (size_t)rows * cb_plen[a] * sizeof(float), hipMemcpyHostToDevice, s));
    AGZ_HIP_TRY(hipMemcpyAsync(d_value[a], h_value[a], (size_t)rows * sizeof(float), hipMemcpyHostToDevice, s));
  }
  return AGZ_OK;
}

int agz_arena::update_slots() {
  slot_host.resize(G);
  if (!split_nets()) {
    for (int g = 0; g < G; g++) slot_host[g] = g;
    nA_slots = G; nB_slots = G;
  } else {
    std::vector<int32_t> tm(G), ab(G);
    AGZ_HIP_TRY(hipMemcpyAsync(tm.data(), d.to_move, G * sizeof(int32_t), hipMemcpyDeviceToHost, ctx->stream));
    AGZ_HIP_TRY(hipMemcpyAsync(ab.data(), d.a_is_black, G * sizeof(int32_t), hipMemcpyDeviceToHost, ctx->stream));
    AGZ_HIP_TRY(hipStreamSynchronize(ctx->stream));
    int na = 0;
    for (int g = 0; g < G; g++) { bool a_moves = (tm[g] == AGZ_BLACK) == (ab[g] != 0); if (a_moves) na++; }
    int ia = 0, ib = na;
    for (int g = 0; g < G; g++) { bool a_moves = (tm[g] == AGZ_BLACK) == (ab[g] != 0); slot_host[g] = a_moves ? ia++ : ib++; }
    nA_slots = na; nB_slots = G - na;
  }
  AGZ_HIP_TRY(hipMemcpyAsync(d.slot_of_game, slot_host.data(), G * sizeof(int32_t), hipMemcpyHostToDevice, ctx->stream));
  AGZ_HIP_TRY(hipStreamSynchronize(ctx->stream));
  return AGZ_OK;
}

int agz_arena::nn_step(int prep, int nl) {
  float* act0 = nullptr; float* act1 = nullptr;
  const size_t slot_elems = (size_t)(gc.m + 2) * (gc.n + 2) * 32;
  if (inf_kind[0] == AGZ_INF_NET) act0 = net[0]->d_act_in;
  if (inf_kind[1] == AGZ_INF_NET) act1 = split_nets() ? net[1]->d_act_in : (net[1]->d_act_in);
  if (split_nets()) {  }
  const bool split_lanes = d.V > 1;
  {
    ProfScope ps(ctx, AGZ_PROF_SELECT);
    if (split_lanes) {
      hipLaunchKernelGGL(k_select_paths, dim3(G), dim3(64), 0, ctx->stream, d, gc, mc, prep, nl);
      hipLaunchKernelGGL(k_leaf, dim3(G * nl), dim3(64), 0, ctx->stream, d, gc, mc, act0, act1, prep, nl);
    } else {
      hipLaunchKernelGGL(k_select, dim3(G), dim3(64), 0, ctx->stream, d, gc, mc, act0, act1, prep, nl);
    }
  }
  bool need_forward = true;
  int prep_batch = 0;
  if (prep) {
    unsigned long long cnt = 0;
    AGZ_HIP_TRY(hipMemcpyAsync(&cnt, d.counters + CNT_PREP_EXPAND, 8, hipMemcpyDeviceToHost, ctx->stream));
    AGZ_HIP_TRY(hipStreamSynchronize(ctx->stream));
    need_forward = cnt != prep_expand_seen;
    const unsigned long long n_need = cnt - prep_expand_seen;
    prep_expand_seen = cnt;
    last_prep_roots = (int)n_need; last_prep_batch = need_forward ? G : 0;
    if (need_forward && prep_compact && !split_nets() && nl == 1 && inf_kind[0] == AGZ_INF_NET && inf_kind[1] == AGZ_INF_NET && n_need < (unsigned long long)G) {
      const int nb = net[0]->min_same_batch((int)n_need, G);
      if (nb < G) {
        const int slot_f4 = (int)(slot_elems / 4);
        hipLaunchKernelGGL(k_prep_compact, dim3(ceil_div(slot_f4, 256)), dim3(256), 0, ctx->stream, d, act0, slot_f4);
        prep_batch = nb; last_prep_batch = nb;
      }
    }
  }
  Dev dx = d;
  if (prep_batch > 0) dx.slot_of_game = d.prep_slot;
  InfDesc inf{};
  for (int a = 0; a < 2; a++) {
    inf.kind[a] = inf_kind[a];
    inf.policy[a] = d_policy[a]; inf.value[a] = d_value[a];
    inf.dummy_player[a] = 0;
    switch (inf_kind[a]) {
      case AGZ_INF_NET: inf.policy_len[a] = net[a]->conf.ActionSpace; break;
      case AGZ_INF_DUMMY: inf.policy_len[a] = gc.A; break;
      case AGZ_INF_SCRIPT: inf.policy_len[a] = 10; break;
      case AGZ_INF_HASH: inf.policy_len[a] = gc.A + 1; break;
      case AGZ_INF_CALLBACK: inf.kind[a] = AGZ_INF_NET; inf.policy_len[a] = cb_plen[a]; break;
      default: inf.policy_len[a] = 25; break;
    }
  }
  if (!need_forward) {
    if (inf_kind[0] == AGZ_INF_NET && inf_kind[1] == AGZ_INF_NET && !split_nets()) { inf.policy[1] = d_policy[0]; inf.value[1] = d_value[0]; }
  } else if (!split_nets()) {
    agz_net* n = inf_kind[0] == AGZ_INF_NET ? net[0] : (inf_kind[1] == AGZ_INF_NET ? net[1] : nullptr);
    if (n) {
      int a = inf_kind[0] == AGZ_INF_NET ? 0 : 1;
      int r = n->forward_packed(prep_batch > 0 ? prep_batch : G * nl, d_policy[a], d_value[a]);
      if (r != AGZ_OK) return r;
      if (inf_kind[0] == AGZ_INF_NET && inf_kind[1] == AGZ_INF_NET) { inf.policy[1] = d_policy[0]; inf.value[1] = d_value[0]; }
    }
  } else {
    if (nA_slots > 0) { int r = net[0]->forward_packed(nA_slots, d_policy[0], d_value[0]); if (r != AGZ_OK) return r; }
    if (nB_slots > 0) {
      agz_net* nb = net[1];
      float* save = nb->d_act_in;
      nb->d_act_in = save + (size_t)nA_slots * slot_elems;
      int r = nb->forward_packed(nB_slots, d_policy[1] + (size_t)nA_slots * nb->conf.ActionSpace, d_value[1] + nA_slots);
      nb->d_act_in = save;
      if (r != AGZ_OK) return r;
    }
  }
  if (d.cb_mask && need_forward) { int r = cb_run(nl); if (r != AGZ_OK) return r; }
  {
    ProfScope ps(ctx, AGZ_PROF_EXPAND);
    if (split_lanes) {
      hipLaunchKernelGGL(k_expand_prep, dim3(G * nl), dim3(64), 0, ctx->stream, dx, gc, mc, inf, nl);
      hipLaunchKernelGGL(k_expand_commit, dim3(G), dim3(64), 0, ctx->stream, dx, gc, mc, prep, nl);
    } else {
      hipLaunchKernelGGL(k_expand, dim3(G), dim3(64), 0, ctx->stream, dx, gc, mc, inf, prep, nl);
    }
  }
  AGZ_HIP_TRY(hipGetLastError());
  return AGZ_OK;
}

__global__ void k_gather_rows(float* __restrict__ dst, const float* __restrict__ src, const int32_t* __restrict__ idx, int n, int rowlen) {
  const size_t g = (size_t)blockIdx.x * 256 + threadIdx.x;
  if (g >= (size_t)n * rowlen) return;
  const int r = (int)(g / rowlen), c = (int)(g - (size_t)r * rowlen);
  dst[(size_t)r * rowlen + c] = src[(size_t)idx[r] * rowlen + c];
}

extern "C" {

int agz_arena_create(agz_ctx* ctx, const agz_game_conf* game, const agz_mcts_conf* mcts, int n_games, uint64_t seed,
                     int max_nodes, agz_arena** out) {
  AGZ_REQUIRE(ctx && game && mcts && out, AGZ_E_INVALID, "agz_arena_create: NULL argument");
  AGZ_REQUIRE(n_games >= 1, AGZ_E_INVALID, "agz_arena_create: n_games must be >= 1");
  AGZ_REQUIRE(mcts->PUCT > 0 && mcts->PUCT <= 1, AGZ_E_INVALID, "MCTSConf is not valid (PUCT must be in (0,1], tree.go:42-44)");
  AGZ_REQUIRE(game->kind >= 0 && game->kind <= 3, AGZ_E_INVALID, "agz_arena_create: unknown game kind %d", game->kind);
  AGZ_REQUIRE(game->m >= 1 && game->n >= 1 && game->m * game->n <= 361, AGZ_E_UNSUPPORTED, "board %dx%d unsupported (max 361 cells)", game->m, game->n);
  if (game->kind == AGZ_GAME_KOMI || game->kind == AGZ_GAME_WQ)
    AGZ_REQUIRE(game->m == game->n, AGZ_E_UNSUPPORTED, "komi/wq boards must be square on device (the reference's non-square geometry is degenerate, game/naughty.go:9-19)");
  AGZ_REQUIRE(game->encoder == AGZ_ENC_TWOPLANE || game->encoder == AGZ_ENC_WQ, AGZ_E_INVALID, "unknown encoder");
  AGZ_REQUIRE(mcts->Budget >= 0, AGZ_E_INVALID, "Budget must be >= 0");
  AGZ_HIP_TRY(hipSetDevice(ctx->device));
  agz_arena* a = new agz_arena();
  a->ctx = ctx; a->G = n_games; a->seed = seed; a->seed0 = seed;
  a->pool_grow = max_nodes <= 0;
  GameCfg& c = a->gc;
  c.kind = game->kind; c.m = game->m; c.n = game->n; c.k = game->k; c.cells = c.m * c.n;
  c.A = c.kind == AGZ_GAME_C4 ? c.n : c.cells;
  c.max_moves = game->max_moves > 0 ? game->max_moves : 2 * c.cells;
  c.encoder = game->encoder; c.F = c.encoder == AGZ_ENC_WQ ? 18 : 2;
  c.komi = game->komi;
  c.flip_in_tree = c.kind != AGZ_GAME_C4;
  c.pass_legal = (c.kind == AGZ_GAME_WQ || c.kind == AGZ_GAME_C4);
  c.go_like = (c.kind == AGZ_GAME_KOMI || c.kind == AGZ_GAME_WQ);
  c.has_passes = c.kind == AGZ_GAME_WQ;
  MctsCfg& m = a->mc;
  m.PUCT = mcts->PUCT; m.maxDepth = mcts->M * mcts->N; m.RandomCount = mcts->RandomCount; m.Budget = mcts->Budget;
  m.RandomMinVisits = mcts->RandomMinVisits; m.RandomTemperature = mcts->RandomTemperature; m.DumbPass = mcts->DumbPass;
  m.ResignPercentage = mcts->ResignPercentage; m.PassPreference = mcts->PassPreference;
  AGZ_REQUIRE(m.maxDepth + 2 <= MAXPATH, AGZ_E_UNSUPPORTED, "M*N too large");
  Dev& d = a->d;
  const int G = n_games, T = 2 * G;
  d.G = G; d.T = T;
  const long long size_by = mcts->Budget > 0 ? mcts->Budget : (n_games == 1 ? 65536 : 0);
  long long cap = max_nodes > 0 ? max_nodes : (long long)(4 * (size_by + 2)) * (c.A + 1) + 16;
  if (cap > 8000000) cap = 8000000;
  d.cap = (int)cap;
  d.moves_stride = c.max_moves + 4;
  int r = AGZ_OK;
#define AL(p, n) if ((r = a->alloc(&d.p, (size_t)(n))) != AGZ_OK) { agz_arena_destroy(a); return r; }
  AL(board, (size_t)G * CELLS_PAD) AL(ring, (size_t)G * RING * CELLS_PAD) AL(to_move, G) AL(ply, G) AL(passes, G)
  AL(pass_count, G) AL(ended, G) AL(winner, G) AL(a_is_black, G) AL(last_move, G) AL(cap_b, G) AL(cap_w, G) AL(zhash, G)
  AL(moves, (size_t)G * d.moves_stride) AL(amoves, (size_t)G * d.moves_stride) AL(n_amoves, G) AL(hist_from, G)
  size_t pool = (size_t)T * 2 * d.cap;
  AL(prior, pool) AL(visits, pool) AL(bsum, pool) AL(kids_off, pool) AL(kids_n, pool) AL(nmove, pool)
  AL(n_nodes, T) AL(cur_pool, T) AL(has_root, T) AL(has_prev, T) AL(prev_ply, T) AL(prev_board, (size_t)T * CELLS_PAD)
  AL(stalled, T) AL(overflow, T) AL(pc_hash, (size_t)T * d.moves_stride) AL(pc_move, (size_t)T * d.moves_stride) AL(pc_n, T) AL(rng, T) AL(rng_game, G)
  d.V = 1;
  AL(vl, pool)
  AL(slot_of_game, G) AL(prep_slot, G) AL(leaf_kind, G) AL(leaf_player, G) AL(leaf_ply, G) AL(leaf_result, G) AL(leaf_board, (size_t)G * CELLS_PAD)
  AL(leaf_legal, (size_t)G * CELLS_PAD) AL(path, (size_t)G * MAXPATH) AL(path_len, G) AL(counters, CNT_N)
  {
    size_t per_ex = (size_t)c.F * c.cells + (c.A + 1) + 3;
    size_t want = std::max<size_t>((size_t)G * c.max_moves * 2, 16384);
    size_t budget = (size_t)(12ull << 30) / (per_ex * 4);
    d.ex_cap = (int)std::min(want, budget);
  }
  AL(ex_planes, (size_t)d.ex_cap * c.F * c.cells) AL(ex_policy, (size_t)d.ex_cap * (c.A + 1)) AL(ex_value, d.ex_cap)
  AL(ex_game, d.ex_cap) AL(ex_prev, d.ex_cap) AL(ex_last, G) AL(ex_count, 1) AL(ex_labelled, d.ex_cap) AL(best_out, G)
  {
    std::vector<int32_t> zt((size_t)2 * c.cells, 0);
    SplitMix64 rr(1337);
    int lim = c.kind == AGZ_GAME_KOMI ? std::min(c.cells + 1, 2 * c.cells) : 2 * c.cells;
    for (int i = 0; i < lim; i++) zt[i] = rr.int31();
    int32_t* zp = nullptr;
    if ((r = a->alloc(&zp, zt.size())) != AGZ_OK) { agz_arena_destroy(a); return r; }
    if (hipMemcpyAsync(zp, zt.data(), zt.size() * sizeof(int32_t), hipMemcpyHostToDevice, ctx->stream) != hipSuccess ||
        hipStreamSynchronize(ctx->stream) != hipSuccess) {
// ... 93 lines not shown
  RL(leaf_kind, n) RL(leaf_player, n) RL(leaf_ply, n) RL(leaf_result, n) RL(leaf_board, n * CELLS_PAD) RL(leaf_legal, n * CELLS_PAD)
  RL(path, n * MAXPATH) RL(path_len, n)
  RL(exp_score, n * CELLS_PAD) RL(exp_move, n * CELLS_PAD) RL(exp_n, n) RL(exp_value, n)
#undef RL
  d.V = lanes;
  AGZ_HIP_TRY(hipStreamSynchronize(a->ctx->stream));
  for (int agent = 0; agent < 2; agent++)
    if (a->inf_kind[agent] == AGZ_INF_NET) { r = agz_arena_set_inferencer(a, agent, AGZ_INF_NET, a->net[agent]); if (r != AGZ_OK) return r; }
  if (a->d.cb_mask) { r = a->cb_setup(); if (r != AGZ_OK) return r; }
  return AGZ_OK;
}

int agz_arena_reset(agz_arena* a, const uint8_t* a_is_black) {
  AGZ_REQUIRE(a, AGZ_E_INVALID, "arena is NULL");
  AGZ_HIP_TRY(hipSetDevice(a->ctx->device));
  hipStream_t s = a->ctx->stream;
  uint8_t* dab = nullptr;
  if (a_is_black) {
    AGZ_HIP_TRY(hipMalloc(&dab, a->G));
    AGZ_HIP_TRY(hipMemcpyAsync(dab, a_is_black, a->G, hipMemcpyHostToDevice, s));
  }
  AGZ_HIP_TRY(hipMemsetAsync(a->d.counters, 0, CNT_N * sizeof(unsigned long long), s));
  AGZ_HIP_TRY(hipMemsetAsync(a->d.ex_count, 0, sizeof(int32_t), s));
  hipLaunchKernelGGL(k_reset, dim3(a->G), dim3(64), 0, s, a->d, a->gc, dab, (unsigned long long)a->seed, (unsigned long long)a->seed0);
  std::vector<int32_t> ab(a->G);
  AGZ_HIP_TRY(hipMemcpyAsync(ab.data(), a->d.a_is_black, a->G * sizeof(int32_t), hipMemcpyDeviceToHost, s));
  AGZ_HIP_TRY(hipStreamSynchronize(s));
  if (dab) hipFree(dab);
  for (int g = 0; g < a->G; g++) a->a_is_black[g] = (uint8_t)ab[g];
  a->in_move = false; a->moves_done = 0; a->prep_expand_seen = 0;
  a->seed += 0x9E3779B97F4A7C15ull;
  return a->update_slots();
}

int agz_arena_begin_move(agz_arena* a) {
  AGZ_REQUIRE(a, AGZ_E_INVALID, "arena is NULL");
  AGZ_REQUIRE(!a->in_move, AGZ_E_STATE, "agz_arena_begin_move: previous move not ended");
  for (int i = 0; i < 2; i++) AGZ_REQUIRE(a->inf_kind[i] != AGZ_INF_NET || a->net[i], AGZ_E_STATE, "agent %d has no net", i);
  AGZ_HIP_TRY(hipSetDevice(a->ctx->device));
  if (a->split_nets()) { int r = a->update_slots(); if (r != AGZ_OK) return r; }
  {
    ProfScope ps(a->ctx, AGZ_PROF_MOVE);
    hipLaunchKernelGGL(k_begin_move, dim3(a->G), dim3(64), 0, a->ctx->stream, a->d, a->gc, a->mc);
  }
  a->in_move = true;
  a->sims_this_move = 0; a->room_sims = 0;
  if (a->pool_grow) {
    const long long sims = a->mc.Budget > 0 ? a->mc.Budget : 0;
    int r = a->ensure_pool_room(sims);
    if (r != AGZ_OK) { a->in_move = false; return r; }
    a->room_sims = sims;
  }
  return a->nn_step(1);
}

int agz_arena_debug_counter(agz_arena* a, int which, int64_t* value) {
  AGZ_REQUIRE(a && value && which >= 0 && which < CNT_N, AGZ_E_INVALID, "agz_arena_debug_counter: bad argument");
  AGZ_HIP_TRY(hipSetDevice(a->ctx->device));
  unsigned long long v = 0;
  AGZ_HIP_TRY(hipMemcpyAsync(&v, a->d.counters + which, 8, hipMemcpyDeviceToHost, a->ctx->stream));
  AGZ_HIP_TRY(hipStreamSynchronize(a->ctx->stream));
  *value = (int64_t)v;
  return AGZ_OK;
}

int agz_arena_pool_capacity(agz_arena* a, int* nodes_per_pool, int* grows) {
  AGZ_REQUIRE(a && nodes_per_pool && grows, AGZ_E_INVALID, "agz_arena_pool_capacity: NULL argument");
  *nodes_per_pool = a->d.cap; *grows = a->pool_grows;
  return AGZ_OK;
}

int agz_arena_set_prep_compact(agz_arena* a, int on) {
  AGZ_REQUIRE(a, AGZ_E_INVALID, "arena is NULL");
  a->prep_compact = on != 0;
  return AGZ_OK;
}

int agz_arena_last_prep_batch(agz_arena* a, int* boards, int* roots) {
  AGZ_REQUIRE(a && boards && roots, AGZ_E_INVALID, "agz_arena_last_prep_batch: NULL argument");
  *boards = a->last_prep_batch; *roots = a->last_prep_roots;
  return AGZ_OK;
}

int agz_arena_simulate(agz_arena* a, int k) {
  AGZ_REQUIRE(a, AGZ_E_INVALID, "arena is NULL");
  AGZ_REQUIRE(a->in_move, AGZ_E_STATE, "agz_arena_simulate: call agz_arena_begin_move first");
  AGZ_HIP_TRY(hipSetDevice(a->ctx->device));
  if (a->pool_grow && a->sims_this_move + k > a->room_sims) {
    int r = a->ensure_pool_room(k);
    if (r != AGZ_OK) return r;
    a->room_sims = a->sims_this_move + k;
  }
  a->sims_this_move += k;
  for (int done = 0; done < k;) {
    int nl = std::min(a->d.V, k - done);
    int r = a->nn_step(0, nl);
    if (r != AGZ_OK) return r;
    done += nl;
  }
  return AGZ_OK;
}

int agz_arena_end_move(agz_arena* a, int record) {
  AGZ_REQUIRE(a, AGZ_E_INVALID, "arena is NULL");
  AGZ_REQUIRE(a->in_move, AGZ_E_STATE, "agz_arena_end_move: call agz_arena_begin_move first");
  AGZ_HIP_TRY(hipSetDevice(a->ctx->device));
  {
    ProfScope ps(a->ctx, AGZ_PROF_MOVE);
    hipLaunchKernelGGL(k_end_move, dim3(a->G), dim3(64), 0, a->ctx->stream, a->d, a->gc, a->mc, record, a->restart ? 1 : 0, (const int32_t*)nullptr, 0);
  }
  AGZ_HIP_TRY(hipGetLastError());
  a->in_move = false;
  a->moves_done++;
  return AGZ_OK;
}

int agz_arena_apply_moves(agz_arena* a, const int32_t* moves) {
  AGZ_REQUIRE(a && moves, AGZ_E_INVALID, "agz_arena_apply_moves: NULL argument");
  AGZ_REQUIRE(!a->in_move, AGZ_E_STATE, "agz_arena_apply_moves: a search is in progress (call agz_arena_end_move first)");
  AGZ_HIP_TRY(hipSetDevice(a->ctx->device));
  hipStream_t s = a->ctx->stream;
  if (!a->d_forced) AGZ_HIP_TRY(hipMalloc(&a->d_forced, (size_t)a->G * sizeof(int32_t)));
  unsigned long long before = 0, after = 0;
  AGZ_HIP_TRY(hipMemcpyAsync(&before, a->d.counters + CNT_ILLEGAL, 8, hipMemcpyDeviceToHost, s));
  AGZ_HIP_TRY(hipMemcpyAsync(a->d_forced, moves, (size_t)a->G * sizeof(int32_t), hipMemcpyHostToDevice, s));
  AGZ_HIP_TRY(hipStreamSynchronize(s));
  hipLaunchKernelGGL(k_end_move, dim3(a->G), dim3(64), 0, s, a->d, a->gc, a->mc, 0, 0, (const int32_t*)a->d_forced, 0);
  AGZ_HIP_TRY(hipGetLastError());
  AGZ_HIP_TRY(hipMemcpyAsync(&after, a->d.counters + CNT_ILLEGAL, 8, hipMemcpyDeviceToHost, s));
  AGZ_HIP_TRY(hipStreamSynchronize(s));
  a->moves_done++;
  AGZ_REQUIRE(after == before, AGZ_E_INVALID, "agz_arena_apply_moves: %llu illegal move(s) (State.Check failed); those games were left unchanged",
              after - before);
  return AGZ_OK;
}

int agz_arena_get_stats(agz_arena* a, agz_arena_stats* out) {
  AGZ_REQUIRE(a && out, AGZ_E_INVALID, "NULL argument");
  AGZ_HIP_TRY(hipSetDevice(a->ctx->device));
  unsigned long long c[CNT_N];
  std::vector<int32_t> ended(a->G);
  AGZ_HIP_TRY(hipMemcpyAsync(c, a->d.counters, sizeof(c), hipMemcpyDeviceToHost, a->ctx->stream));
  AGZ_HIP_TRY(hipMemcpyAsync(ended.data(), a->d.ended, a->G * sizeof(int32_t), hipMemcpyDeviceToHost, a->ctx->stream));
  AGZ_HIP_TRY(hipStreamSynchronize(a->ctx->stream));
  out->sims_total = (int64_t)c[CNT_SIMS]; out->sims_nonnull = (int64_t)c[CNT_NONNULL]; out->nn_evals = (int64_t)c[CNT_EVALS];
  out->moves_played = (int64_t)c[CNT_MOVES]; out->games_finished = (int64_t)c[CNT_GAMES]; out->examples = (int64_t)c[CNT_EXAMPLES];
  out->n_games = a->G; out->tree_full = (int32_t)c[CNT_FULL]; out->examples_dropped = (int32_t)c[CNT_DROPPED];
  out->path_nodes = (int64_t)c[CNT_PATH]; out->children_read = (int64_t)c[CNT_KIDS];
  int act = 0;
  for (int g = 0; g < a->G; g++) act += ended[g] ? 0 : 1;
  out->n_active = act;
  return AGZ_OK;
}

int agz_arena_get_results(agz_arena* a, int64_t* a_wins, int64_t* b_wins, int64_t* draws) {
  AGZ_REQUIRE(a, AGZ_E_INVALID, "arena is NULL");
  AGZ_HIP_TRY(hipSetDevice(a->ctx->device));
  unsigned long long c[CNT_N];
  AGZ_HIP_TRY(hipMemcpyAsync(c, a->d.counters, sizeof(c), hipMemcpyDeviceToHost, a->ctx->stream));
  AGZ_HIP_TRY(hipStreamSynchronize(a->ctx->stream));
  if (a_wins) *a_wins = (int64_t)c[CNT_A_WINS];
  if (b_wins) *b_wins = (int64_t)c[CNT_B_WINS];
  if (draws) *draws = (int64_t)c[CNT_DRAWS];
  return AGZ_OK;
}

// ... 615 lines not shown
```

### agogo_amd/csrc/net.hip

```cpp
#include "net.hpp"
#include "gemm_maps.hpp"

#include <cmath>
#include <cstdio>
#include <cstring>
#include <type_traits>

typedef float f32x16 __attribute__((ext_vector_type(16)));
typedef float f32x4 __attribute__((ext_vector_type(4)));

namespace agz {

struct ConvArgs {
  const float* x;
  const float* w;
  const void* ep;
  float* y;
  int M, HW, W, Wp, HpWp;
  int Cin_p, Cout_p, Ntot;
  int n_mtiles, n_ntiles;
  int raw;
  int splits;
  int per;
  float* ws;
// ... 953 lines not shown
  }
  AGZ_REQUIRE((int)h_ep_dual.size() == conf.SharedLayers && !h_ep_init.empty(), AGZ_E_STATE, "agz_net: Winograd weights before commit");
  const int hw = H * W;
  std::vector<float> e2;
  for (int l = 0; l < conf.SharedLayers; l++) {
    const std::vector<float>& e = h_ep_dual[l];
    const bool more = l + 1 < conf.SharedLayers;
    e2.assign(e.size(), 0.f);
    for (int p = 0; p < hw; p++)
      for (int c = 0; c < Kp; c++) {
        const float tn = more ? tins[l + 1][c] : 1.0f;
        const size_t o = ((size_t)p * Kp + c) * 4;
        e2[o + 0] = e[o + 0] * coluns[l][c] * tn; e2[o + 1] = e[o + 1] * tn;
        e2[o + 2] = e[o + 2] * coluns[l][Kp + c] * tn; e2[o + 3] = e[o + 3] * tn;
      }
    if (chained) {
      double g1 = 0.0, g0 = 0.0;
      for (int p = 0; p < hw; p++)
        for (int c = 0; c < Kp; c++) {
          const double tn = more ? tins[l + 1][c] : 1.0;
          const size_t o = ((size_t)p * Kp + c) * 4;
          g1 = std::max(g1, tn * (std::fabs((double)e[o + 0]) * l1s[l][c] + std::fabs((double)e[o + 2]) * l1s[l][Kp + c]));
          g0 = std::max(g0, tn * (std::max((double)e[o + 1], 0.0) + std::max((double)e[o + 3], 0.0)));
        }
      wino_g1[l] = (float)(g1 * (1.0 + 1e-6)); wino_g0[l] = (float)(g0 * (1.0 + 1e-6));
    }
    AGZ_HIP_TRY(hipMalloc(&d_ep_h2[l], e2.size() * 4));
    AGZ_HIP_TRY(hipMemcpyAsync(d_ep_h2[l], e2.data(), e2.size() * 4, hipMemcpyHostToDevice, ctx->stream));
    AGZ_HIP_TRY(hipStreamSynchronize(ctx->stream));
  }
  if (conf.SharedLayers > 0) {
    e2.assign(h_ep_init.size(), 0.f);
    for (int p = 0; p < hw; p++)
      for (int c = 0; c < Kp; c++) {
        const size_t o = ((size_t)p * Kp + c) * 2;
        e2[o] = h_ep_init[o] * tins[0][c]; e2[o + 1] = h_ep_init[o + 1] * tins[0][c];
      }
    AGZ_HIP_TRY(hipMalloc(&d_ep_init_h2, e2.size() * 4));
    AGZ_HIP_TRY(hipMemcpyAsync(d_ep_init_h2, e2.data(), e2.size() * 4, hipMemcpyHostToDevice, ctx->stream));
    AGZ_HIP_TRY(hipStreamSynchronize(ctx->stream));
  }
  return AGZ_OK;
}

agz_net::FwdPlan agz_net::fwd_plan(int B) const {
  const int M = B * HW;
  FwdPlan p{};
  auto n_tiles128 = [&](int ntot) { return ceil_div(M, 128) * ceil_div(ntot, 128); };
  p.half_init = cfg == 0 && n_tiles128(Kp) < ctx->num_cus;
  p.half_dual = cfg == 0 && n_tiles128(2 * Kp) < ctx->num_cus;
  const int tiles_dual = cfg != 0 ? ceil_div(M, 128) * ceil_div(2 * Kp, 64) : ceil_div(M, 64) * ceil_div(2 * Kp, 128);
  p.small = latency_mode && Kp >= 64 &&
            (tiles_dual * 4 <= ctx->num_cus || (Kp >= 256 && tiles_dual <= ctx->num_cus));
  p.forced_split = compute_force && cfg == 0 && conf.SharedLayers > 0 &&
                   (this->compute_mode == AGZ_COMPUTE_WINO_H2 || this->compute_mode == AGZ_COMPUTE_WINO ||
                    this->compute_mode == AGZ_COMPUTE_BF16X3 || this->compute_mode == AGZ_COMPUTE_FP16X2);
  p.latency = p.small && !p.forced_split;
  const int spread_max = 64;
  p.heads_spread = p.small || (latency_mode && (B <= spread_max || Kp >= 256));
  p.heads_nb = B >= 32;
  p.split_ok = cfg == 0 && !p.latency && (!p.half_dual || compute_force) && conf.SharedLayers > 0 &&
               (size_t)B * Hp * Wp * Kp * sizeof(float) < ((size_t)1 << 32);
  {
    const int npos = (wino_tm + 2) * (wino_tm + 2), tpb = ceil_div(H, wino_tm) * ceil_div(W, wino_tm);
    p.wino_wide = (2 * Kp) % 256 == 0 && (size_t)npos * ceil_div(B * tpb, 128) * ((2 * Kp) / 256) >= (size_t)ctx->num_cus;
  }
  return p;
}

int agz_net::min_same_batch(int n, int G) const {
  if (n >= G) return G;
  const FwdPlan want = fwd_plan(G);
  auto same = [&](int B) {
    const FwdPlan q = fwd_plan(B);
    return q.half_init == want.half_init && q.half_dual == want.half_dual && q.small == want.small && q.forced_split == want.forced_split &&
           q.latency == want.latency && q.heads_spread == want.heads_spread && q.split_ok == want.split_ok && q.heads_nb == want.heads_nb && q.wino_wide == want.wino_wide;
  };
  if (same(n)) return n;
  for (int B = 16; B < G; B *= 2)
    if (B > n && same(B)) return B;
  return G;
}

int agz_net::forward_packed(int B, float* policy_dev, float* value_dev) {
  AGZ_REQUIRE(committed, AGZ_E_STATE, "agz_net: infer before agz_net_commit");
  AGZ_REQUIRE(B >= 1 && B <= max_batch, AGZ_E_INVALID, "agz_net: batch %d exceeds allocated %d", B, max_batch);
  ConvArgs a{};
  a.M = B * HW; a.HW = HW; a.W = W; a.Wp = Wp; a.HpWp = Hp * Wp;
  a.x = d_act_in; a.w = d_w_init; a.ep = d_ep_init; a.y = d_actA;
  a.Cin_p = Fp; a.Cout_p = Kp; a.Ntot = Kp;
  const FwdPlan plan = fwd_plan(B);
  const bool half_init = plan.half_init, half_dual = plan.half_dual, latency = plan.latency, heads_spread = plan.heads_spread, split_ok = plan.split_ok;
  float** wsp = latency ? &d_ws : nullptr;
  int compute_mode = this->compute_mode;
  if (compute_mode == AGZ_COMPUTE_AUTO) compute_mode = !d_u2_dual.empty() ? AGZ_COMPUTE_WINO_H2 : AGZ_COMPUTE_BF16X3;
  const bool use_h2 = split_ok && compute_mode == AGZ_COMPUTE_FP16X2;
  const bool wino_ok = split_ok && compute_mode == AGZ_COMPUTE_WINO;
  const bool wino_h2_ok = split_ok && compute_mode == AGZ_COMPUTE_WINO_H2;
  if (wino_h2_ok && d_ep_init_h2) a.ep = d_ep_init_h2;
  if (use_h2 && (size_t)B > amax_cap) {
    AGZ_HIP_TRY(hipStreamSynchronize(ctx->stream));
    if (d_amax) hipFree(d_amax);
    d_amax = nullptr; amax_cap = 0;
    AGZ_HIP_TRY(hipMalloc(&d_amax, (size_t)B * sizeof(unsigned)));
    amax_cap = (size_t)B;
  }
  bool lat_h2 = latency && cfg == 0 && this->compute_mode != AGZ_COMPUTE_F32_MFMA && conf.SharedLayers > 0 &&
                (int)d_lat_w2.size() == conf.SharedLayers && agz::conv_lat_ok(Kp, Kp, Wp) && ceil_div(HW, agz::LAT_ROWS) * (Kp / 8) <= 256;
  for (int l = 0; lat_h2 && l < conf.SharedLayers; l++) lat_h2 = d_lat_w2[l] != nullptr;
  const int in_groups = ceil_div(HW, agz::LAT_IN_PIX), in_words = in_groups * (Kp / 64);
  const bool lat_in = lat_h2 && Fp == 32 && Kp % 64 == 0 && in_words <= 256 && d_w_init_t;
  if (lat_h2 && lat_wmax_cap < B) {
    AGZ_HIP_TRY(hipStreamSynchronize(ctx->stream));
    for (auto& p2 : d_lat_wmax) { if (p2) hipFree(p2); p2 = nullptr; }
    lat_wmax_cap = 0;
    for (auto& p2 : d_lat_wmax) AGZ_HIP_TRY(hipMalloc(&p2, (size_t)B * 256 * sizeof(float)));
    lat_wmax_cap = B;
  }
  int rc;
  bool amax0_done = false;
  if (lat_in) {
    agz::LatInArgs li{};
    li.x = d_act_in; li.w = d_w_init_t; li.ep = reinterpret_cast<const float2*>(d_ep_init); li.t = d_lat_tin[0]; li.y = d_actA; li.words = d_lat_wmax[1];
    li.B = B; li.H = H; li.W = W; li.Hp = Hp; li.Wp = Wp; li.Cout_p = Kp; li.groups_per_board = in_groups;
    ProfScope ps(ctx, AGZ_PROF_CONV_INIT);
    hipLaunchKernelGGL(agz::lat_input_kernel, dim3(Kp / 64, B * in_groups), dim3(256), 0, ctx->stream, li);
    rc = AGZ_OK;
  }
  else if (split_ok && compute_mode != AGZ_COMPUTE_F32_MFMA && d_w3_init && Kp % 128 == 0 &&
      (size_t)B * Hp * Wp * Fp * sizeof(float) < ((size_t)1 << 32)) {
    a.n_ntiles = ceil_div(a.Ntot, 128); a.n_mtiles = ceil_div(a.M, 128);
    a.splits = 1; a.per = 0; a.ws = nullptr; a.raw = 0;
    ProfScope ps(ctx, AGZ_PROF_CONV_INIT);
    if (wino_h2_ok && d_amax && amax_cap >= (size_t)B) {
      AGZ_HIP_TRY(hipMemsetAsync(d_amax, 0, (size_t)B * sizeof(unsigned), ctx->stream));
      a.amax_out = d_amax; amax0_done = true;
    }
    hipLaunchKernelGGL((conv3x3_x3_kernel<false>), dim3(a.n_mtiles * a.n_ntiles), dim3(256), 0, ctx->stream, a, d_w3_init);
    a.amax_out = nullptr;
    rc = AGZ_OK;
  }
  else if (cfg != 0) rc = launch_conv<4, 1, 1, false>(ctx, a, wsp, &ws_cap);
  else if (half_init) rc = launch_conv<2, 2, 1, false>(ctx, a, wsp, &ws_cap);
  else rc = launch_conv<2, 2, 2, false>(ctx, a, wsp, &ws_cap);
  if (rc != AGZ_OK) return rc;
  float* cur = d_actA;
  float* nxt = d_actB;
  bool tower_done = false;
  if (!tower_done && wino_h2_ok) {
    AGZ_REQUIRE((int)d_u2_dual.size() == conf.SharedLayers, AGZ_E_STATE, "agz_net: Winograd fp16x2 weights not built");
    const int npos = (wino_tm + 2) * (wino_tm + 2);
    const int tpb = ceil_div(H, wino_tm) * ceil_div(W, wino_tm);
    const bool wide = plan.wino_wide;
    static const int chunk_env = [] { const char* e = getenv("AGZ_WINO_H2_CHUNK"); return e ? atoi(e) : 0; }();
    static const int queues_env = [] { const char* e = getenv("AGZ_WINO_H2_QUEUES"); return e ? atoi(e) : 0; }();
    const int queues_want = queues_env > 0 ? queues_env : (tower_queues > 0 ? tower_queues : (B >= 256 ? 2 : 1));
    const int chunk_max = (int)std::min<size_t>((size_t)B, ((((size_t)1 << 32) - 1) / ((size_t)npos * Kp * 4) - 127) / tpb);
    int chunk = chunk_env >= 1 ? std::min(chunk_env, chunk_max) : chunk_max;
    const int ns = (queues_want == 2 && B >= 64) ? 2 : 1;
    if (ns == 2 && chunk >= B) chunk = (B + 1) / 2;
    const size_t v_elems = wino_h2_rows(npos, (size_t)chunk * tpb) * Kp, m_elems = 2 * v_elems;
    static const int form_env = [] { const char* e = getenv("AGZ_WINO_H2_FORM"); return e ? atoi(e) : -1; }();
    const int form_want = wino_form >= 0 ? wino_form : form_env;
    const bool chained = form_want != 0 && (int)d_u2c_dual.size() == conf.SharedLayers && agz::wino_h2c_ok(H, W, wino_tm, Kp);
    const int n_scr = chained ? ceil_div(B, chunk) : ns;
    if (v_elems * n_scr > wino_v_cap) {
      AGZ_HIP_TRY(hipStreamSynchronize(ctx->stream));
      if (ctx->stream2) AGZ_HIP_TRY(hipStreamSynchronize(ctx->stream2));
      if (d_wV) hipFree(d_wV);
      if (d_wM) hipFree(d_wM);
      d_wV = d_wM = nullptr; wino_chunk_cap = 0;
      AGZ_HIP_TRY(hipMalloc(&d_wV, v_elems * n_scr * sizeof(float)));
      AGZ_HIP_TRY(hipMalloc(&d_wM, m_elems * n_scr * sizeof(float)));
      wino_v_cap = v_elems * n_scr; wino_chunk_cap = 0;
    }
    const size_t wm_board = chained ? (size_t)tpb * (Kp >> 5) * 2 : (size_t)tpb * (Kp >> 6);
    const size_t need_amax = (size_t)(conf.SharedLayers + 1) * B + wm_board * B;
    if (need_amax > amax_cap) {
      AGZ_HIP_TRY(hipStreamSynchronize(ctx->stream));
      if (ctx->stream2) AGZ_HIP_TRY(hipStreamSynchronize(ctx->stream2));
      if (d_amax) hipFree(d_amax);
      d_amax = nullptr; amax_cap = 0;
      AGZ_HIP_TRY(hipMalloc(&d_amax, need_amax * sizeof(unsigned)));
      amax_cap = need_amax;
      amax0_done = false;
    }
    float* d_wave_max = reinterpret_cast<float*>(d_amax + (size_t)(conf.SharedLayers + 1) * B);
    if (!amax0_done)
      hipLaunchKernelGGL(board_amax_kernel, dim3(B), dim3(256), 0, ctx->stream, cur, d_amax, HW, W, Wp, Hp * Wp, Kp, (const float*)nullptr);
    if (ns == 2) {
      if (!ctx->stream2) {
        AGZ_HIP_TRY(hipStreamCreateWithFlags(&ctx->stream2, hipStreamNonBlocking));
        AGZ_HIP_TRY(hipEventCreateWithFlags(&ctx->ev_fork, hipEventDisableTiming));
        AGZ_HIP_TRY(hipEventCreateWithFlags(&ctx->ev_join, hipEventDisableTiming));
      }
      AGZ_HIP_TRY(hipEventRecord(ctx->ev_fork, ctx->stream));
      AGZ_HIP_TRY(hipStreamWaitEvent(ctx->stream2, ctx->ev_fork, 0));
    }
    for (int l = 0; chained && l < conf.SharedLayers; l++) {
      ProfScope ps(ctx, AGZ_PROF_CONV);
      int ci = 0;
      const size_t wmb = (size_t)tpb * (Kp >> 5);
      const bool last = l + 1 == conf.SharedLayers;
      for (int b0 = 0; b0 < B; b0 += chunk, ci++) {
        const int q = ci % ns;
        hipStream_t st = q ? ctx->stream2 : ctx->stream;
        WinoH2Args hh{};
        WinoArgs& wa = hh.w;
        wa.x = cur + (size_t)b0 * Hp * Wp * Kp; wa.y = nxt + (size_t)b0 * Hp * Wp * Kp;
        wa.V = d_wV + (size_t)ci * v_elems; wa.Mb = d_wM + (size_t)ci * m_elems; wa.ep = d_ep_h2[l];
        wa.B = std::min(chunk, B - b0); wa.H = H; wa.W = W; wa.Hp = Hp; wa.Wp = Wp; wa.C = Kp; wa.Cout_p = Kp; wa.Ntot = 2 * Kp;
        hh.U2c = d_u2c_dual[l]; hh.w_unscale = 1.f; hh.tm = wino_tm;
        hh.amax_in = d_amax + (size_t)l * B + b0;
        hh.amax_next = last ? nullptr : d_amax + (size_t)(l + 1) * B + b0;
        hh.amax_true = l == 0 ? reinterpret_cast<const float*>(d_amax + b0) : nullptr;
        hh.wm_prev = d_wave_max + ((size_t)((l + 1) & 1) * B + b0) * wmb;
        hh.wm_out = d_wave_max + ((size_t)(l & 1) * B + b0) * wmb;
        hh.g1 = wino_g1[l]; hh.g0 = wino_g0[l];
        {
          static const int gemm_env = [] {
            const char* e = getenv("AGZ_WINO_H2_GEMM");
            const int v = e ? atoi(e) : 0;
            if (v == 0 || (((v & 63) == 1 || (v & 63) == 2) && (v >> 6) <= 1)) return v;
            fprintf(stderr, "libagz: AGZ_WINO_H2_GEMM=%s ignored (want 1 or 2, optionally + 64)\n", e);
            return 0;
          }();
          const int gv = wino_gemm > 0 ? wino_gemm : gemm_env;
          hh.gemm_variant = gv & 63; hh.temporal_stores = (gv >> 6) & 1;
        }
        if (l == 0) agz::wino_h2c_in(ctx, hh, st);
        agz::wino_h2c_gemm(ctx, hh, st);
        agz::wino_h2c_oi(ctx, hh, last, st, form_want == 1 ? 1 : 4);
      }
      if (last) std::swap(cur, nxt);
    }
    for (int l = 0; !chained && l < conf.SharedLayers; l++) {
      ProfScope ps(ctx, AGZ_PROF_CONV);
      int ci = 0;
      for (int b0 = 0; b0 < B; b0 += chunk, ci++) {
        const int q = ci % ns;
        WinoH2Args hh{};
        WinoArgs& wa = hh.w;
        wa.x = cur + (size_t)b0 * Hp * Wp * Kp; wa.y = nxt + (size_t)b0 * Hp * Wp * Kp;
        wa.V = d_wV + (size_t)q * v_elems; wa.Mb = d_wM + (size_t)q * m_elems; wa.ep = d_ep_h2[l];
        wa.B = std::min(chunk, B - b0); wa.H = H; wa.W = W; wa.Hp = Hp; wa.Wp = Wp; wa.C = Kp; wa.Cout_p = Kp; wa.Ntot = 2 * Kp;
        hh.U2 = d_u2_dual[l]; hh.w_unscale = 1.f; hh.tm = wino_tm;
        hh.t_in = nullptr; hh.col_unscale = nullptr; hh.t_next = nullptr;
        hh.amax_in = d_amax + (size_t)l * B + b0; hh.amax_out = d_amax + (size_t)(l + 1) * B + b0;
        hh.wave_max = d_wave_max + (size_t)b0 * wm_board;
        hh.fuse_prev = l > 0;
        wino_h2_launch(ctx, hh, wide, q ? ctx->stream2 : ctx->stream);
      }
      std::swap(cur, nxt);
    }
    if (ns == 2) {
      AGZ_HIP_TRY(hipEventRecord(ctx->ev_join, ctx->stream2));
      AGZ_HIP_TRY(hipStreamWaitEvent(ctx->stream, ctx->ev_join, 0));
    }
    tower_done = true;
  }
  for (int l = 0; !tower_done && l < conf.SharedLayers; l++) {
    a.x = cur; a.w = d_w_dual[l]; a.ep = d_ep_dual[l]; a.y = nxt;
    a.Cin_p = Kp; a.Cout_p = Kp; a.Ntot = 2 * Kp;
    if (use_h2) {
      a.n_ntiles = ceil_div(a.Ntot, 128); a.n_mtiles = ceil_div(a.M, 128);
      a.splits = 1; a.per = 0; a.ws = nullptr; a.raw = 0;
      hipLaunchKernelGGL(board_amax_kernel, dim3(B), dim3(256), 0, ctx->stream, cur, d_amax, HW, W, Wp, Hp * Wp, Kp);
      a.amax_in = d_amax; a.w_unscale = w_unscale[l];
      ProfScope ps(ctx, AGZ_PROF_CONV);
      if ((2 * Kp) % 256 == 0) {
        a.n_ntiles = (2 * Kp) / 256;
        hipLaunchKernelGGL(conv3x3_h2w_kernel, dim3(a.n_mtiles * a.n_ntiles), dim3(256), 0, ctx->stream, a, d_w2_dual[l]);
      } else {
        hipLaunchKernelGGL(conv3x3_h2_kernel, dim3(a.n_mtiles * a.n_ntiles), dim3(256), 0, ctx->stream, a, d_w2_dual[l]);
      }
      rc = AGZ_OK;
    }
    else if (wino_ok) {
      AGZ_REQUIRE((int)d_u3_dual.size() == conf.SharedLayers && d_u3_dual[l], AGZ_E_STATE, "agz_net: Winograd weights not built");
      static const int chunk_env = [] { const char* e = getenv("AGZ_WINO_CHUNK"); return e ? atoi(e) : 0; }();
      const int tpb = ceil_div(H, 4) * ceil_div(W, 4);
      const int chunk_max = (int)std::min<size_t>((size_t)B, (((size_t)1 << 32) - 1) / ((size_t)36 * tpb * Kp * 4));
      const int chunk = chunk_env >= 1 ? std::min(chunk_env, chunk_max) : chunk_max;
      if (chunk > wino_chunk_cap) {
        AGZ_HIP_TRY(hipStreamSynchronize(ctx->stream));
        if (d_wV) hipFree(d_wV);
        if (d_wM) hipFree(d_wM);
        d_wV = d_wM = nullptr; wino_chunk_cap = 0;
        AGZ_HIP_TRY(hipMalloc(&d_wV, (size_t)36 * chunk * tpb * Kp * sizeof(float)));
        AGZ_HIP_TRY(hipMalloc(&d_wM, (size_t)36 * chunk * tpb * 2 * Kp * sizeof(float)));
        wino_chunk_cap = chunk; wino_v_cap = 0;
      }
      ProfScope ps(ctx, AGZ_PROF_CONV);
      for (int b0 = 0; b0 < B; b0 += chunk) {
        WinoArgs wa{};
        wa.x = cur + (size_t)b0 * Hp * Wp * Kp; wa.y = nxt + (size_t)b0 * Hp * Wp * Kp;
        wa.V = d_wV; wa.Mb = d_wM; wa.U3 = d_u3_dual[l]; wa.ep = d_ep_dual[l];
        wa.B = std::min(chunk, B - b0); wa.H = H; wa.W = W; wa.Hp = Hp; wa.Wp = Wp; wa.C = Kp; wa.Cout_p = Kp; wa.Ntot = 2 * Kp;
        wino_launch(ctx, wa, WINO_IN | WINO_GEMM | WINO_OUT);
      }
      rc = AGZ_OK;
    }
    else if (split_ok && compute_mode == AGZ_COMPUTE_BF16X3) {
      a.n_ntiles = ceil_div(a.Ntot, 128); a.n_mtiles = ceil_div(a.M, 128);
      a.splits = 1; a.per = 0; a.ws = nullptr; a.raw = 0;
      ProfScope ps(ctx, AGZ_PROF_CONV);
      hipLaunchKernelGGL((conv3x3_x3_kernel<true>), dim3(a.n_mtiles * a.n_ntiles), dim3(256), 0, ctx->stream, a, d_w3_dual[l]);
      rc = AGZ_OK;
    }
    else if (lat_h2) {
      const int gpb = ceil_div(HW, agz::LAT_ROWS), words = gpb * (Kp / 8);
      agz::LatH2Args la{};
      la.x = cur; la.w2 = d_lat_w2[l]; la.t_in = d_lat_tin[l]; la.col_unscale = d_lat_colun[l]; la.ep = d_ep_dual[l]; la.y = nxt;
      la.B = B; la.H = H; la.W = W; la.Hp = Hp; la.Wp = Wp; la.C = Kp; la.Cout_p = Kp; la.Ntot = 2 * Kp;
      la.groups_per_board = gpb;
      if (l == 0) {
        if (!lat_in) hipLaunchKernelGGL(agz::lat_board_words_kernel, dim3(B * 64), dim3(256), 0, ctx->stream, cur, (const float*)d_lat_tin[0], d_lat_wmax[1], HW, W, Wp, Hp * Wp, Kp, 64);
        la.wmax_in = d_lat_wmax[1]; la.n_in_words = lat_in ? in_words : 64;
      } else {
        la.wmax_in = d_lat_wmax[(l - 1) & 1]; la.n_in_words = words;
      }
      const bool more = l + 1 < conf.SharedLayers;
      la.t_next = more ? d_lat_tin[l + 1] : nullptr;
      la.wmax_out = more ? d_lat_wmax[l & 1] : nullptr;
      ProfScope ps(ctx, AGZ_PROF_CONV);
      agz::conv_lat_h2_launch(ctx, la);
      rc = AGZ_OK;
    }
    else if (cfg != 0) rc = launch_conv<4, 1, 1, true>(ctx, a, wsp, &ws_cap);
    else if (half_dual) rc = launch_conv<2, 2, 1, true>(ctx, a, wsp, &ws_cap);
    else rc = launch_conv<2, 2, 2, true>(ctx, a, wsp, &ws_cap);
    if (rc != AGZ_OK) return rc;
    std::swap(cur, nxt);
  }
  HeadArgs h{};
  h.x = cur; h.conv = d_head_conv; h.bn = d_head_bn; h.Wp = d_Wp; h.bp = d_bp; h.W1 = d_W1; h.b1 = d_b1; h.W2 = d_W2;
  h.b2 = d_b2; h.policy = policy_dev; h.value = value_dev;
  h.H = H; h.W = W; h.HW = HW; h.Wp_ = Wp; h.HpWp = Hp * Wp; h.Kp = Kp; h.A = conf.ActionSpace; h.FC = conf.FC;
  size_t smem = (size_t)(3 * HW + 8 + conf.FC) * sizeof(float);
  {
    ProfScope ps(ctx, AGZ_PROF_HEADS);
    if (heads_spread) {
      size_t need = (size_t)B * (3 * HW + conf.ActionSpace + conf.FC);
      if (need > hs_cap) {
        AGZ_HIP_TRY(hipStreamSynchronize(ctx->stream));
        if (d_hs) hipFree(d_hs);
        d_hs = nullptr; hs_cap = 0;
        AGZ_HIP_TRY(hipMalloc(&d_hs, need * sizeof(float)));
        hs_cap = need;
      }
      h.feat = d_hs; h.cols = d_hs + (size_t)B * 3 * HW;
      hipLaunchKernelGGL(heads_feat_kernel, dim3(ceil_div(HW, 4), B), dim3(256), 0, ctx->stream, h);
      if (plan.heads_nb)
        hipLaunchKernelGGL(heads_fc_nb_kernel<4>, dim3(ceil_div(conf.ActionSpace + conf.FC, 64), ceil_div(B, 4)), dim3(1024), 0, ctx->stream, h, B);
      else
        hipLaunchKernelGGL(heads_fc_kernel, dim3(ceil_div(conf.ActionSpace + conf.FC, 64), B), dim3(1024), 0, ctx->stream, h);
      hipLaunchKernelGGL(heads_out_kernel, dim3(B), dim3(256), 0, ctx->stream, h);
    } else {
      hipLaunchKernelGGL(heads_kernel, dim3(B), dim3(256), smem, ctx->stream, h);
    }
  }
  AGZ_HIP_TRY(hipGetLastError());
  return AGZ_OK;
}

int agz_net::forward_dev(const float* planes_dev, int B, float* policy_dev, float* value_dev) {
  AGZ_REQUIRE(committed, AGZ_E_STATE, "agz_net: infer before agz_net_commit");
  int r = ensure_batch(B);
  if (r != AGZ_OK) return r;
  int total = B * HW * Fp;
  hipLaunchKernelGGL(pack_planes_kernel, dim3(ceil_div(total, 256)), dim3(256), 0, ctx->stream, planes_dev, d_act_in, B,
                     conf.Features, H, W, Fp);
  return forward_packed(B, policy_dev, value_dev);
}

extern "C" {

int agz_net_create(agz_ctx* ctx, const agz_net_conf* c, agz_net** out) {
  AGZ_REQUIRE(ctx && c && out, AGZ_E_INVALID, "agz_net_create: NULL argument");
  AGZ_REQUIRE(c->K >= 1 && c->ActionSpace >= 3 && c->SharedLayers >= 0 && c->FC > 1 && c->BatchSize >= 1 && c->Features > 0,
              AGZ_E_INVALID, "agz_net_create: NNConf is not valid");
  AGZ_REQUIRE(c->Width >= 1 && c->Height >= 1, AGZ_E_INVALID, "agz_net_create: bad board size");
  AGZ_REQUIRE(c->Features <= 32, AGZ_E_UNSUPPORTED, "agz_net_create: Features > 32 unsupported");
  AGZ_REQUIRE(c->ActionSpace <= 512, AGZ_E_UNSUPPORTED, "agz_net_create: ActionSpace > 512 unsupported");
  AGZ_REQUIRE(c->bn_mode >= 0 && c->bn_mode <= 2, AGZ_E_INVALID, "agz_net_create: bad bn_mode");
  agz_net* n = new agz_net();
  n->ctx = ctx;
  n->conf = *c;
  n->H = c->Height; n->W = c->Width; n->HW = n->H * n->W; n->Hp = n->H + 2; n->Wp = n->W + 2;
  n->Kp = round_up(c->K, 32);
  n->cfg = (n->Kp % 64 == 0) ? 0 : 1;
  int K = c->K, F = c->Features, H = n->H, W = n->W, hw = n->HW, B = c->BatchSize;
  auto conv = [&](const std::string& nm, int o, int i, int k) {
    n->params.push_back(Param{"Filter" + nm, std::vector<float>((size_t)o * i * k * k, 0.f), {o, i, k, k}, 0});
  };
  auto bnp = [&](const std::string& nm, int C) {
    n->params.push_back(Param{nm + "_gamma", std::vector<float>((size_t)C * hw, 0.f), {B, C, H, W}, 1});
    n->params.push_back(Param{nm + "_beta", std::vector<float>((size_t)C * hw, 0.f), {B, C, H, W}, 1});
    n->bn.push_back(BNStats{std::vector<float>(C, 0.f), std::vector<float>(C, 1.f)});
  };
  auto fc = [&](const std::string& nm, int in, int units) {
    n->params.push_back(Param{nm + "_w", std::vector<float>((size_t)in * units, 0.f), {in, units}, 2});
    n->params.push_back(Param{nm + "_b", std::vector<float>((size_t)units, 0.f), {B, units}, 3});
  };
  conv("Init", K, F, 3); bnp("Init", K);
  for (int i = 0; i < c->SharedLayers; i++) {
    std::string s = std::to_string(i);
    conv("Layer1 of Shared Layer " + s, K, K, 3); bnp("L1_" + s, K);
    conv("Layer2 of Shared Layer " + s, K, K, 3); bnp("L2_" + s, K);
  }
  conv("PolicyHead", 2, K, 1); bnp("PolicyHead", 2);
  fc("Policy", 2 * hw, c->ActionSpace);
  conv("ValueHead", 1, K, 1); bnp("ValueHead", 1);
  fc("Value", hw, c->FC);
  fc("ValueOutput", c->FC, 1);
  *out = n;
  return AGZ_OK;
}

void agz_net_destroy(agz_net* n) {
  if (!n) return;
  hipStreamSynchronize(n->ctx->stream);
  n->free_device();
  delete n;
}

int agz_net_num_params(const agz_net* n) { return n ? (int)n->params.size() : 0; }

int agz_net_param_info(const agz_net* n, int i, char* name, size_t cap, size_t* n_elems) {
  AGZ_REQUIRE(n && i >= 0 && i < (int)n->params.size(), AGZ_E_INVALID, "agz_net_param_info: bad index %d", i);
  if (name && cap) { strncpy(name, n->params[i].name.c_str(), cap - 1); name[cap - 1] = 0; }
  if (n_elems) *n_elems = n->params[i].v.size();
  return AGZ_OK;
}

int agz_net_set_param(agz_net* n, int i, const float* host, size_t cnt) {
  AGZ_REQUIRE(n && host && i >= 0 && i < (int)n->params.size(), AGZ_E_INVALID, "agz_net_set_param: bad argument");
  Param& p = n->params[i];
  if (p.kind == 1 && cnt == (size_t)p.ref_shape[1]) {
    int C = p.ref_shape[1], hw = n->HW;
// ... 438 lines not shown
```

### agogo_amd/csrc/net.hpp

```cpp
#pragma once
#include <string>
#include <vector>

#include "common.hpp"

namespace agz {
struct Param {
  std::string name;
  std::vector<float> v;
  std::vector<int> ref_shape;
  int kind;
};
struct BNStats { std::vector<float> mean, var; };
int conv3x3_raw(agz_ctx* ctx, const float* x, const float* w, float* y, int B, int H, int W, int Cin_p, int Cout_p);
int conv3x3_raw_x3(agz_ctx* ctx, const float* x, const unsigned short* w3, float* y, int B, int H, int W, int Cin_p, int Cout_p);
int split_w3(agz_ctx* ctx, const float* w, unsigned short* w3, int N, int Cin_p);
inline size_t w3_elems(int N, int Cin_p) { return (size_t)9 * 3 * N * Cin_p; }
struct WinoRawScratch {
  float* V = nullptr; float* M = nullptr; void* U2 = nullptr; unsigned* words = nullptr;
  size_t v_cap = 0, m_cap = 0, u_cap = 0; int b_cap = 0;
  void* w2 = nullptr; unsigned* h2_words = nullptr;
  size_t w2_cap = 0; int h2_b_cap = 0, h2_flip = 0;
};
int conv3x3_raw_h2(agz_ctx* ctx, const float* x, const float* w, float* y, int B, int H, int W, int Cin_p, int Cout_p, WinoRawScratch* sc,
                   const unsigned* ranges = nullptr);
bool conv3x3_raw_h2_fits(int B, int H, int W, int Cin_p, int Cout_p);
int conv3x3_raw_h2_weights(agz_ctx* ctx, const float* w, int Cin_p, int Cout_p, WinoRawScratch* sc, const void** w2, const unsigned** w_amax);
struct RawWeights { void* img = nullptr; unsigned* words = nullptr; size_t cap = 0; };
int conv3x3_raw_h2_weights_to(agz_ctx* ctx, hipStream_t st, const float* w, int Cin_p, int Cout_p, RawWeights* out);
int conv3x3_raw_wino_h2_weights_to(agz_ctx* ctx, hipStream_t st, const float* w, int H, int W, int Cin_p, int Cout_p, RawWeights* out);
void raw_weights_free(RawWeights* rw);
int conv3x3_raw_wino_h2(agz_ctx* ctx, const float* x, const float* w, float* y, int B, int H, int W, int Cin_p, int Cout_p, WinoRawScratch* sc,
                        const unsigned* ranges = nullptr, const RawWeights* pre = nullptr);
bool conv3x3_raw_wino_h2_fits(int B, int H, int W, int Cin_p, int Cout_p);
void wino_raw_scratch_free(WinoRawScratch* sc);
}

struct agz_net {
  agz_ctx* ctx = nullptr;
  agz_net_conf conf{};
  std::vector<agz::Param> params;
  std::vector<agz::BNStats> bn;
  bool committed = false;

  int H = 0, W = 0, HW = 0, Hp = 0, Wp = 0;
  int Kp = 0;
  int Fp = 32;
  int cfg = 0;

  float* d_w_init = nullptr;
  float* d_w_init_t = nullptr;
  float* d_ep_init = nullptr;
  unsigned short* d_w3_init = nullptr;
  std::vector<float*> d_w_dual;
  std::vector<float*> d_ep_dual;
  std::vector<unsigned short*> d_w3_dual;
  std::vector<_Float16*> d_w2_dual;
  std::vector<float> w_unscale;
  std::vector<unsigned short*> d_u3_dual;
  std::vector<_Float16*> d_u2_dual;
  std::vector<float> u_unscale;
  std::vector<float*> d_u2_tin;
  std::vector<float*> d_u2_colun;
  std::vector<_Float16*> d_u2c_dual;
  std::vector<float> wino_g1, wino_g0;
  int wino_gemm = 0;
  int wino_form = -1;
  void free_u2c() { for (auto& p : d_u2c_dual) if (p) hipFree(p); d_u2c_dual.clear(); wino_g1.clear(); wino_g0.clear(); }
  int build_wino_h2_weights();
  int wino_tm = 4;
  size_t wino_v_cap = 0;
  float* d_wV = nullptr;
  float* d_wM = nullptr;
  int wino_chunk_cap = 0;
  int build_wino_weights();
  unsigned* d_amax = nullptr;
  size_t amax_cap = 0;
  int compute_mode = AGZ_COMPUTE_F32_MFMA;
  bool compute_force = false;
  float* d_head_conv = nullptr;
  float* d_head_bn = nullptr;
  float* d_Wp = nullptr;
  float* d_bp = nullptr;
  float* d_W1 = nullptr;
  float* d_b1 = nullptr;
  float* d_W2 = nullptr;
  float* d_b2 = nullptr;

  int max_batch = 0;
  float* d_act_in = nullptr;
  float* d_actA = nullptr;
  float* d_actB = nullptr;
  float* d_planes = nullptr;
  float* d_policy = nullptr;
  float* d_value = nullptr;
  float* d_ws = nullptr;
  std::vector<std::vector<float>> h_ep_dual;
  std::vector<float> h_ep_init;
  std::vector<float*> d_ep_h2;
  float* d_ep_init_h2 = nullptr;
  std::vector<_Float16*> d_lat_w2;
  std::vector<float*> d_lat_tin, d_lat_colun;
  float* d_lat_wmax[2] = {nullptr, nullptr};
  int lat_wmax_cap = 0;
  size_t ws_cap = 0;
  float* d_hs = nullptr;
  size_t hs_cap = 0;
  int tower_queues = 0;
  bool latency_mode = true;

  int ensure_batch(int B);
  void free_device();
  int forward_dev(const float* planes_dev, int B, float* policy_dev, float* value_dev);
  int forward_packed(int B, float* policy_dev, float* value_dev);
  struct FwdPlan { bool half_init, half_dual, small, forced_split, latency, heads_spread, split_ok, heads_nb, wino_wide; };
  FwdPlan fwd_plan(int B) const;
  int min_same_batch(int n, int G) const;
};
```

### include/agz_debug.h

```cpp
#ifndef AGZ_DEBUG_H
#define AGZ_DEBUG_H

#include "agz.h"

#ifdef __cplusplus
extern "C" {
#endif

#define AGZ_PROF_CONV 0
#define AGZ_PROF_HEADS 1
#define AGZ_PROF_SELECT 2
#define AGZ_PROF_EXPAND 3
#define AGZ_PROF_MOVE 4
#define AGZ_PROF_CONV_INIT 5
#define AGZ_PROF_WINO_IN 6
#define AGZ_PROF_WINO_GEMM 7
#define AGZ_PROF_WINO_OUT 8
#define AGZ_PROF_NCLASS 9
int agz_ctx_prof_enable(agz_ctx* ctx, int enable);
int agz_ctx_prof_read(agz_ctx* ctx, int klass, int64_t* launches, double* total_ms);
int agz_ctx_prof_set_stride(agz_ctx* ctx, int klass, int stride);

int agz_wino_stages(agz_ctx* ctx, const float* x, const float* w, int B, int H, int W, int C, int N, float* V, float* M);

int agz_wino_h2_tile(int H, int W);

int agz_wino_h2_chained(int H, int W, int K);

int agz_net_set_wino_h2_form(agz_net* net, int form);

int agz_net_set_wino_h2_gemm(agz_net* net, int variant);

int agz_arena_set_prep_compact(agz_arena* arena, int on);
int agz_arena_last_prep_batch(agz_arena* arena, int* boards, int* roots);

int agz_trainer_set_dma_forward(agz_trainer* t, int on);

int agz_net_min_same_batch(agz_net* net, int n, int G, int* batch);

#define AGZ_CNT_PATHMAX 15
int agz_arena_debug_counter(agz_arena* arena, int which, int64_t* value);

int agz_arena_pool_capacity(agz_arena* arena, int* nodes_per_pool, int* grows);

int agz_comm_debug_fail_slice(agz_comm* comm, int k);

int agz_comm_debug_fail_layer(agz_comm* comm, int layer);

#ifdef __cplusplus
}
#endif
#endif
```

Baseline: 42460.

## Split MCTS step into two half-batches pipelined across two streams

Each arena step (select, network forward, expand) is split into two halves of the games, each run on its own stream with events, so one half's tree kernels can overlap the other half's network forward. The main stream becomes a wrapper that lazily joins the secondary stream whenever it is used elsewhere. The Winograd tower and heads code is refactored into per-half helpers. This adds event and launch overhead and halves the GEMM batch size, which may lower GPU utilisation.

```diff
diff --git a/agogo_amd/capi.py b/agogo_amd/capi.py
--- a/agogo_amd/capi.py
+++ b/agogo_amd/capi.py
@@ -219,6 +219,8 @@
     sig("agz_net_set_wino_h2_gemm", i32, vp, i32)
     sig("agz_net_min_same_batch", i32, vp, i32, i32, C.POINTER(C.c_int))
     sig("agz_arena_set_prep_compact", i32, vp, i32)
+    sig("agz_arena_set_split", i32, vp, i32)
+    sig("agz_arena_split_steps", i32, vp, C.POINTER(C.c_int64), C.POINTER(C.c_int64), C.POINTER(C.c_int))
     sig("agz_trainer_set_dma_forward", i32, vp, i32)
     sig("agz_arena_last_prep_batch", i32, vp, C.POINTER(C.c_int), C.POINTER(C.c_int))
     sig("agz_arena_debug_counter", i32, vp, i32, C.POINTER(C.c_int64))
@@ -699,6 +701,14 @@
     def set_prep_compact(self, on=True):
         _check(lib().agz_arena_set_prep_compact(self.h, int(on)), "agz_arena_set_prep_compact")
 
+    def set_split(self, mode=1):
+        _check(lib().agz_arena_set_split(self.h, int(mode)), "agz_arena_set_split")
+
+    def split_steps(self):
+        s_, j_, l_ = C.c_int64(0), C.c_int64(0), C.c_int(0)
+        _check(lib().agz_arena_split_steps(self.h, C.byref(s_), C.byref(j_), C.byref(l_)), "agz_arena_split_steps")
+        return s_.value, j_.value, bool(l_.value)
+
     def last_prep_batch(self):
         b, r = C.c_int(0), C.c_int(0)
         _check(lib().agz_arena_last_prep_batch(self.h, C.byref(b), C.byref(r)), "agz_arena_last_prep_batch")
diff --git a/agogo_amd/csrc/common.hpp b/agogo_amd/csrc/common.hpp
--- a/agogo_amd/csrc/common.hpp
+++ b/agogo_amd/csrc/common.hpp
@@ -40,16 +40,31 @@
 
 }
 
+struct agz_ctx;
+namespace agz {
+struct MainStream {
+  agz_ctx* c = nullptr;
+  hipStream_t s = nullptr;
+  inline operator hipStream_t() const;
+  hipStream_t raw() const { return s; }
+};
+}
+
 struct agz_ctx {
   int device = 0;
-  hipStream_t stream = nullptr;
+  agz::MainStream stream;
   hipStream_t stream2 = nullptr;
   hipEvent_t ev_fork = nullptr, ev_join = nullptr;
+  hipEvent_t ev_mid[2] = {nullptr, nullptr};
+  bool open2 = false;
+  const void* open_owner = nullptr;
+  int ensure_stream2();
+  void join();
   bool prof_on = false;
   unsigned prof_mask = ~0u;
   int prof_stride[AGZ_PROF_NCLASS];
   int64_t prof_seen[AGZ_PROF_NCLASS] = {};
-  agz_ctx() { for (auto& v : prof_stride) v = 1; }
+  agz_ctx() { for (auto& v : prof_stride) v = 1; stream.c = this; }
   agz::ProfClass prof[AGZ_PROF_NCLASS];
   int prof_open = 0;
   int num_cus = 256;
@@ -59,6 +74,8 @@
   void prof_end(int klass);
   int prof_collect();
 };
+
+inline agz::MainStream::operator hipStream_t() const { if (c->open2) c->join(); return s; }
 
 namespace agz {
 struct ProfScope {
diff --git a/agogo_amd/csrc/conv_wino_h2.hpp b/agogo_amd/csrc/conv_wino_h2.hpp
--- a/agogo_amd/csrc/conv_wino_h2.hpp
+++ b/agogo_amd/csrc/conv_wino_h2.hpp
@@ -1098,13 +1098,13 @@
   h.fuse_prev = (h.fuse_prev && fuse) ? 1 : 0;
   h.amax_self = const_cast<unsigned*>(h.amax_in);
   {
-    ProfScopeOn ps(ctx, AGZ_PROF_WINO_IN, st == ctx->stream);
+    ProfScopeOn ps(ctx, AGZ_PROF_WINO_IN, st == ctx->stream.raw());
     const size_t n_in = (size_t)a.T * (a.C / 2);
     if (tm == 5) hipLaunchKernelGGL(wino_in_h2_kernel<5>, dim3((unsigned)((n_in + 255) / 256)), dim3(256), 0, st, h);
     else hipLaunchKernelGGL(wino_in_h2_kernel<4>, dim3((unsigned)((n_in + 255) / 256)), dim3(256), 0, st, h);
   }
   {
-    ProfScopeOn ps(ctx, AGZ_PROF_WINO_GEMM, st == ctx->stream);
+    ProfScopeOn ps(ctx, AGZ_PROF_WINO_GEMM, st == ctx->stream.raw());
     const dim3 gw(h.npos * a.n_mtiles * ceil_div(a.Ntot, 256)), gn(h.npos * a.n_mtiles * a.n_ntiles);
     const int nk = a.C >> 5;
     bool done = true;
@@ -1125,7 +1125,7 @@
     else hipLaunchKernelGGL(wino_gemm_h2_kernel, gn, dim3(256), 0, st, h);
   }
   {
-    ProfScopeOn ps(ctx, AGZ_PROF_WINO_OUT, st == ctx->stream);
+    ProfScopeOn ps(ctx, AGZ_PROF_WINO_OUT, st == ctx->stream.raw());
     const size_t n_out = (size_t)a.T * a.Cout_p;
     if (h.raw) {
       const unsigned bd = a.Ntot % 256 == 0 ? 256u : (a.Ntot % 128 == 0 ? 128u : (a.Ntot % 64 == 0 ? 64u : 32u));
diff --git a/agogo_amd/csrc/conv_wino_h2c.hpp b/agogo_amd/csrc/conv_wino_h2c.hpp
--- a/agogo_amd/csrc/conv_wino_h2c.hpp
+++ b/agogo_amd/csrc/conv_wino_h2c.hpp
@@ -802,7 +802,7 @@
 static void wino_h2c_in(agz_ctx* ctx, WinoH2Args& h, hipStream_t st) {
   wino_h2c_geometry(h);
   h.fuse_prev = 0; h.amax_self = const_cast<unsigned*>(h.amax_in);
-  ProfScopeOn ps(ctx, AGZ_PROF_WINO_IN, st == ctx->stream);
+  ProfScopeOn ps(ctx, AGZ_PROF_WINO_IN, st == ctx->stream.raw());
   const size_t n_in = (size_t)h.w.T * (h.w.C / 2);
   if (h.tm == 5) hipLaunchKernelGGL(wino_in_h2_kernel<5>, dim3((unsigned)((n_in + 255) / 256)), dim3(256), 0, st, h);
   else hipLaunchKernelGGL(wino_in_h2_kernel<4>, dim3((unsigned)((n_in + 255) / 256)), dim3(256), 0, st, h);
@@ -810,7 +810,7 @@
 constexpr int WINO_H2_GEMM_DEFAULT = 1;
 static void wino_h2c_gemm(agz_ctx* ctx, WinoH2Args& h, hipStream_t st) {
   wino_h2c_geometry(h);
-  ProfScopeOn ps(ctx, AGZ_PROF_WINO_GEMM, st == ctx->stream);
+  ProfScopeOn ps(ctx, AGZ_PROF_WINO_GEMM, st == ctx->stream.raw());
   const dim3 g(h.npos * h.w.n_mtiles * (h.w.Ntot >> 8));
   const bool dma_ok = wino_h2_rows(h.npos, (size_t)h.w.T) * h.w.C * 4 < ((size_t)1 << 31) && (size_t)h.npos * h.w.C * h.w.Ntot * 4 < ((size_t)1 << 31);
   const int variant_all = h.gemm_variant > 0 ? h.gemm_variant : WINO_H2_GEMM_DEFAULT;
@@ -844,7 +844,7 @@
 }
 static void wino_h2c_oi(agz_ctx* ctx, WinoH2Args& h, bool last, hipStream_t st, int variant = 4) {
   wino_h2c_geometry(h);
-  ProfScopeOn ps(ctx, AGZ_PROF_WINO_OUT, st == ctx->stream);
+  ProfScopeOn ps(ctx, AGZ_PROF_WINO_OUT, st == ctx->stream.raw());
   const WinoArgs& a = h.w;
   const dim3 g((unsigned)ceil_div(a.T, 16), (unsigned)(a.C >> 5));
   const size_t shm = last ? 0 : (size_t)(16 / a.TPB) * a.H * a.W * 32 * sizeof(float);
diff --git a/agogo_amd/csrc/ctx.hip b/agogo_amd/csrc/ctx.hip
--- a/agogo_amd/csrc/ctx.hip
+++ b/agogo_amd/csrc/ctx.hip
@@ -28,6 +28,22 @@
   p.used++;
   if (prof_open > 0) prof_open--;
   if (p.used >= 4096 && prof_open == 0) prof_collect();
+}
+int agz_ctx::ensure_stream2() {
+  if (stream2) return AGZ_OK;
+  AGZ_HIP_TRY(hipStreamCreateWithFlags(&stream2, hipStreamNonBlocking));
+  AGZ_HIP_TRY(hipEventCreateWithFlags(&ev_fork, hipEventDisableTiming));
+  AGZ_HIP_TRY(hipEventCreateWithFlags(&ev_join, hipEventDisableTiming));
+  for (auto& e : ev_mid) AGZ_HIP_TRY(hipEventCreateWithFlags(&e, hipEventDisableTiming));
+  return AGZ_OK;
+}
+void agz_ctx::join() {
+  if (!open2) return;
+  open2 = false; open_owner = nullptr;
+  if (hipEventRecord(ev_join, stream2) != hipSuccess || hipStreamWaitEvent(stream.s, ev_join, 0) != hipSuccess) {
+    (void)hipGetLastError();
+    hipStreamSynchronize(stream2);
+  }
 }
 int agz_ctx::prof_collect() {
   AGZ_HIP_TRY(hipStreamSynchronize(stream));
@@ -66,7 +82,7 @@
   hipDeviceProp_t prop;
   AGZ_HIP_TRY(hipGetDeviceProperties(&prop, device));
   c->num_cus = prop.multiProcessorCount;
-  AGZ_HIP_TRY(hipStreamCreateWithFlags(&c->stream, hipStreamNonBlocking));
+  AGZ_HIP_TRY(hipStreamCreateWithFlags(&c->stream.s, hipStreamNonBlocking));
   *out = c;
   return AGZ_OK;
 }
@@ -91,17 +107,20 @@
 void agz_ctx_destroy(agz_ctx* c) {
   if (!c) return;
   hipSetDevice(c->device);
+  c->join();
   hipStreamSynchronize(c->stream);
   for (auto& p : c->prof)
     for (auto& pr : p.pairs) { hipEventDestroy(pr.first); hipEventDestroy(pr.second); }
   if (c->stream2) hipStreamDestroy(c->stream2);
   if (c->ev_fork) hipEventDestroy(c->ev_fork);
   if (c->ev_join) hipEventDestroy(c->ev_join);
+  for (auto e : c->ev_mid) if (e) hipEventDestroy(e);
   hipStreamDestroy(c->stream);
   delete c;
 }
 int agz_ctx_sync(agz_ctx* c) {
   AGZ_REQUIRE(c, AGZ_E_INVALID, "ctx is NULL");
+  c->join();
   AGZ_HIP_TRY(hipStreamSynchronize(c->stream));
   return AGZ_OK;
 }
diff --git a/agogo_amd/csrc/engine.hip b/agogo_amd/csrc/engine.hip
--- a/agogo_amd/csrc/engine.hip
+++ b/agogo_amd/csrc/engine.hip
@@ -383,9 +383,9 @@
   if (lane == 0) d.has_prev[t] = 0;
 }
 
-__global__ __launch_bounds__(64) void k_select(Dev d, GameCfg c, MctsCfg mc, float* act_in0, float* act_in1, int prep, int nl) {
+__global__ __launch_bounds__(64) void k_select(Dev d, GameCfg c, MctsCfg mc, float* act_in0, float* act_in1, int prep, int nl, int g0) {
   __shared__ Sh s;
-  int g = blockIdx.x, lane = threadIdx.x;
+  int g = g0 + blockIdx.x, lane = threadIdx.x;
   const size_t q0 = (size_t)g * d.V;
   if (d.ended[g]) { if (lane < nl) d.leaf_kind[q0 + lane] = LEAF_NONE; return; }
   int agent = agent_of(d, g);
@@ -703,9 +703,9 @@
   if (n_lanes > 0 && n_null == n_lanes && lane == 0) d.stalled[t] = 1;
 }
 
-__global__ __launch_bounds__(64) void k_expand(Dev d, GameCfg c, MctsCfg mc, InfDesc inf, int prep, int nl) {
+__global__ __launch_bounds__(64) void k_expand(Dev d, GameCfg c, MctsCfg mc, InfDesc inf, int prep, int nl, int g0) {
   __shared__ Sh s;
-  int g = blockIdx.x, lane = threadIdx.x;
+  int g = g0 + blockIdx.x, lane = threadIdx.x;
   if (d.ended[g]) return;
   int agent = agent_of(d, g);
   int t = agent * d.G + g;
@@ -1255,6 +1255,11 @@
   int cb_run(int nl);
   int update_slots();
   int nn_step(int prep, int nl = 1);
+  int split_mode = 1;
+  bool last_step_split = false;
+  int64_t split_steps = 0, joined_steps = 0;
+  bool split_eligible() const;
+  int nn_step_split();
 };
 
 __global__ __launch_bounds__(256) void k_prep_compact(Dev d, float* act, int slot_f4) {
@@ -1436,7 +1441,49 @@
   return AGZ_OK;
 }
 
+bool agz_arena::split_eligible() const {
+  if (split_mode == 0 || d.V != 1 || d.cb_mask != 0 || (G & 1)) return false;
+  if (inf_kind[0] != AGZ_INF_NET || inf_kind[1] != AGZ_INF_NET || net[0] != net[1] || !net[0]) return false;
+  if (ctx->prof_on && (ctx->prof_mask & ((1u << AGZ_PROF_NCLASS) - 1u) & ~(1u << AGZ_PROF_MOVE))) return false;
+  return net[0]->half_ok(G);
+}
+
+int agz_arena::nn_step_split() {
+  agz_net* n = net[0];
+  const int h = G / 2;
+  int r = ctx->ensure_stream2();
+  if (r != AGZ_OK) return r;
+  if (ctx->open2 && ctx->open_owner != this) ctx->join();
+  r = n->forward_half_reserve(G);
+  if (r != AGZ_OK) return r;
+  InfDesc inf{};
+  for (int a = 0; a < 2; a++) {
+    inf.kind[a] = AGZ_INF_NET; inf.policy[a] = d_policy[0]; inf.value[a] = d_value[0];
+    inf.dummy_player[a] = 0; inf.policy_len[a] = n->conf.ActionSpace;
+  }
+  const bool first = !ctx->open2;
+  const bool hold = split_mode == 2;
+  hipStream_t q[2] = {first ? (hipStream_t)ctx->stream : ctx->stream.raw(), ctx->stream2};
+  float* act = n->d_act_in;
+  for (int k = 0; k < 2; k++) {
+    if (k == 1 && (first || hold)) AGZ_HIP_TRY(hipStreamWaitEvent(q[1], ctx->ev_mid[0], 0));
+    if (k == 0 && hold && !first) AGZ_HIP_TRY(hipStreamWaitEvent(q[0], ctx->ev_mid[1], 0));
+    hipLaunchKernelGGL(k_select, dim3(h), dim3(64), 0, q[k], d, gc, mc, act, act, 0, 1, k * h);
+    r = n->forward_half(G, k, q[k], d_policy[0], d_value[0], (k == 0 && (first || hold)) || (k == 1 && hold) ? ctx->ev_mid[k] : nullptr);
+    if (r != AGZ_OK) { ctx->open2 = true; ctx->open_owner = this; ctx->join(); return r; }
+    hipLaunchKernelGGL(k_expand, dim3(h), dim3(64), 0, q[k], d, gc, mc, inf, 0, 1, k * h);
+    if (k == 0) { ctx->open2 = true; ctx->open_owner = this; }
+  }
+  AGZ_HIP_TRY(hipGetLastError());
+  return AGZ_OK;
+}
+
 int agz_arena::nn_step(int prep, int nl) {
+  if (prep == 0 && nl == 1 && split_eligible()) {
+    last_step_split = true; split_steps++;
+    return nn_step_split();
+  }
+  if (!prep) { last_step_split = false; joined_steps++; }
   float* act0 = nullptr; float* act1 = nullptr;
   const size_t slot_elems = (size_t)(gc.m + 2) * (gc.n + 2) * 32;
   if (inf_kind[0] == AGZ_INF_NET) act0 = net[0]->d_act_in;
@@ -1449,7 +1496,7 @@
       hipLaunchKernelGGL(k_select_paths, dim3(G), dim3(64), 0, ctx->stream, d, gc, mc, prep, nl);
       hipLaunchKernelGGL(k_leaf, dim3(G * nl), dim3(64), 0, ctx->stream, d, gc, mc, act0, act1, prep, nl);
     } else {
-      hipLaunchKernelGGL(k_select, dim3(G), dim3(64), 0, ctx->stream, d, gc, mc, act0, act1, prep, nl);
+      hipLaunchKernelGGL(k_select, dim3(G), dim3(64), 0, ctx->stream, d, gc, mc, act0, act1, prep, nl, 0);
     }
   }
   bool need_forward = true;
@@ -1515,7 +1562,7 @@
       hipLaunchKernelGGL(k_expand_prep, dim3(G * nl), dim3(64), 0, ctx->stream, dx, gc, mc, inf, nl);
       hipLaunchKernelGGL(k_expand_commit, dim3(G), dim3(64), 0, ctx->stream, dx, gc, mc, prep, nl);
     } else {
-      hipLaunchKernelGGL(k_expand, dim3(G), dim3(64), 0, ctx->stream, dx, gc, mc, inf, prep, nl);
+      hipLaunchKernelGGL(k_expand, dim3(G), dim3(64), 0, ctx->stream, dx, gc, mc, inf, prep, nl, 0);
     }
   }
   AGZ_HIP_TRY(hipGetLastError());
@@ -1775,6 +1822,21 @@
   return AGZ_OK;
 }
 
+int agz_arena_set_split(agz_arena* a, int mode) {
+  AGZ_REQUIRE(a && mode >= 0 && mode <= 2, AGZ_E_INVALID, "agz_arena_set_split: mode 0 (joined), 1 (split) or 2 (split, skew held)");
+  a->ctx->join();
+  a->split_mode = mode;
+  return AGZ_OK;
+}
+
+int agz_arena_split_steps(agz_arena* a, int64_t* split, int64_t* joined, int* last_split) {
+  AGZ_REQUIRE(a, AGZ_E_INVALID, "arena is NULL");
+  if (split) *split = a->split_steps;
+  if (joined) *joined = a->joined_steps;
+  if (last_split) *last_split = a->last_step_split ? 1 : 0;
+  return AGZ_OK;
+}
+
 int agz_arena_simulate(agz_arena* a, int k) {
   AGZ_REQUIRE(a, AGZ_E_INVALID, "arena is NULL");
   AGZ_REQUIRE(a->in_move, AGZ_E_STATE, "agz_arena_simulate: call agz_arena_begin_move first");
diff --git a/agogo_amd/csrc/net.hip b/agogo_amd/csrc/net.hip
--- a/agogo_amd/csrc/net.hip
+++ b/agogo_amd/csrc/net.hip
@@ -1059,6 +1059,149 @@
   return G;
 }
 
+agz_net::H2Tower agz_net::wino_h2_tower(int B) const {
+  H2Tower t{};
+  t.npos = (wino_tm + 2) * (wino_tm + 2);
+  t.tpb = ceil_div(H, wino_tm) * ceil_div(W, wino_tm);
+  static const int chunk_env = [] { const char* e = getenv("AGZ_WINO_H2_CHUNK"); return e ? atoi(e) : 0; }();
+  static const int queues_env = [] { const char* e = getenv("AGZ_WINO_H2_QUEUES"); return e ? atoi(e) : 0; }();
+  const int queues_want = queues_env > 0 ? queues_env : (tower_queues > 0 ? tower_queues : (B >= 256 ? 2 : 1));
+  const int chunk_max = (int)std::min<size_t>((size_t)B, ((((size_t)1 << 32) - 1) / ((size_t)t.npos * Kp * 4) - 127) / t.tpb);
+  t.chunk = chunk_env >= 1 ? std::min(chunk_env, chunk_max) : chunk_max;
+  t.ns = (queues_want == 2 && B >= 64) ? 2 : 1;
+  if (t.ns == 2 && t.chunk >= B) t.chunk = (B + 1) / 2;
+  t.v_elems = wino_h2_rows(t.npos, (size_t)t.chunk * t.tpb) * Kp; t.m_elems = 2 * t.v_elems;
+  static const int form_env = [] { const char* e = getenv("AGZ_WINO_H2_FORM"); return e ? atoi(e) : -1; }();
+  t.form_want = wino_form >= 0 ? wino_form : form_env;
+  t.chained = t.form_want != 0 && (int)d_u2c_dual.size() == conf.SharedLayers && agz::wino_h2c_ok(H, W, wino_tm, Kp);
+  t.n_scr = t.chained ? ceil_div(B, t.chunk) : t.ns;
+  t.wm_board = t.chained ? (size_t)t.tpb * (Kp >> 5) * 2 : (size_t)t.tpb * (Kp >> 6);
+  return t;
+}
+
+int agz_net::wino_h2_reserve(int B, const H2Tower& t, bool* amax_moved) {
+  if (t.v_elems * t.n_scr > wino_v_cap) {
+    AGZ_HIP_TRY(hipStreamSynchronize(ctx->stream));
+    if (ctx->stream2) AGZ_HIP_TRY(hipStreamSynchronize(ctx->stream2));
+    if (d_wV) hipFree(d_wV);
+    if (d_wM) hipFree(d_wM);
+    d_wV = d_wM = nullptr; wino_chunk_cap = 0;
+    AGZ_HIP_TRY(hipMalloc(&d_wV, t.v_elems * t.n_scr * sizeof(float)));
+    AGZ_HIP_TRY(hipMalloc(&d_wM, t.m_elems * t.n_scr * sizeof(float)));
+    wino_v_cap = t.v_elems * t.n_scr; wino_chunk_cap = 0;
+  }
+  const size_t need_amax = (size_t)(conf.SharedLayers + 1) * B + t.wm_board * B;
+  if (need_amax > amax_cap) {
+    AGZ_HIP_TRY(hipStreamSynchronize(ctx->stream));
+    if (ctx->stream2) AGZ_HIP_TRY(hipStreamSynchronize(ctx->stream2));
+    if (d_amax) hipFree(d_amax);
+    d_amax = nullptr; amax_cap = 0;
+    AGZ_HIP_TRY(hipMalloc(&d_amax, need_amax * sizeof(unsigned)));
+    amax_cap = need_amax;
+    if (amax_moved) *amax_moved = true;
+  }
+  return AGZ_OK;
+}
+
+void agz_net::wino_h2c_block(int l, int B, int b0, int ci, const H2Tower& t, hipStream_t st, float* cur, float* nxt) {
+  const size_t wmb = (size_t)t.tpb * (Kp >> 5);
+  const bool last = l + 1 == conf.SharedLayers;
+  float* d_wave_max = reinterpret_cast<float*>(d_amax + (size_t)(conf.SharedLayers + 1) * B);
+  WinoH2Args hh{};
+  WinoArgs& wa = hh.w;
+  wa.x = cur + (size_t)b0 * Hp * Wp * Kp; wa.y = nxt + (size_t)b0 * Hp * Wp * Kp;
+  wa.V = d_wV + (size_t)ci * t.v_elems; wa.Mb = d_wM + (size_t)ci * t.m_elems; wa.ep = d_ep_h2[l];
+  wa.B = std::min(t.chunk, B - b0); wa.H = H; wa.W = W; wa.Hp = Hp; wa.Wp = Wp; wa.C = Kp; wa.Cout_p = Kp; wa.Ntot = 2 * Kp;
+  hh.U2c = d_u2c_dual[l]; hh.w_unscale = 1.f; hh.tm = wino_tm;
+  hh.amax_in = d_amax + (size_t)l * B + b0;
+  hh.amax_next = last ? nullptr : d_amax + (size_t)(l + 1) * B + b0;
+  hh.amax_true = l == 0 ? reinterpret_cast<const float*>(d_amax + b0) : nullptr;
+  hh.wm_prev = d_wave_max + ((size_t)((l + 1) & 1) * B + b0) * wmb;
+  hh.wm_out = d_wave_max + ((size_t)(l & 1) * B + b0) * wmb;
+  hh.g1 = wino_g1[l]; hh.g0 = wino_g0[l];
+  {
+    static const int gemm_env = [] {
+      const char* e = getenv("AGZ_WINO_H2_GEMM");
+      const int v = e ? atoi(e) : 0;
+      if (v == 0 || (((v & 63) == 1 || (v & 63) == 2) && (v >> 6) <= 1)) return v;
+      fprintf(stderr, "libagz: AGZ_WINO_H2_GEMM=%s ignored (want 1 or 2, optionally + 64)\n", e);
+      return 0;
+    }();
+    const int gv = wino_gemm > 0 ? wino_gemm : gemm_env;
+    hh.gemm_variant = gv & 63; hh.temporal_stores = (gv >> 6) & 1;
+  }
+  if (l == 0) agz::wino_h2c_in(ctx, hh, st);
+  agz::wino_h2c_gemm(ctx, hh, st);
+  agz::wino_h2c_oi(ctx, hh, last, st, t.form_want == 1 ? 1 : 4);
+}
+
+void agz_net::heads_spread_range(agz::HeadArgs h, bool nb4, int B, int b0, int nb, hipStream_t st) {
+  h.x += (size_t)b0 * Hp * Wp * Kp;
+  h.feat = d_hs + (size_t)b0 * 3 * HW; h.cols = d_hs + (size_t)B * 3 * HW + (size_t)b0 * (conf.ActionSpace + conf.FC);
+  h.policy += (size_t)b0 * conf.ActionSpace; h.value += b0;
+  hipLaunchKernelGGL(heads_feat_kernel, dim3(ceil_div(HW, 4), nb), dim3(256), 0, st, h);
+  if (nb4)
+    hipLaunchKernelGGL(heads_fc_nb_kernel<4>, dim3(ceil_div(conf.ActionSpace + conf.FC, 64), ceil_div(nb, 4)), dim3(1024), 0, st, h, nb);
+  else
+    hipLaunchKernelGGL(heads_fc_kernel, dim3(ceil_div(conf.ActionSpace + conf.FC, 64), nb), dim3(1024), 0, st, h);
+  hipLaunchKernelGGL(heads_out_kernel, dim3(nb), dim3(256), 0, st, h);
+}
+
+bool agz_net::half_ok(int B) const {
+  if (!committed || B < 2 || B > max_batch || (B & 1) || (B / 2) % 4 != 0 || cfg != 0 || conf.SharedLayers <= 0) return false;
+  if (min_same_batch(B / 2, B) != B / 2) return false;
+  const FwdPlan plan = fwd_plan(B);
+  int mode = compute_mode;
+  if (mode == AGZ_COMPUTE_AUTO) mode = !d_u2_dual.empty() ? AGZ_COMPUTE_WINO_H2 : AGZ_COMPUTE_BF16X3;
+  if (!plan.split_ok || plan.latency || mode != AGZ_COMPUTE_WINO_H2 || !plan.heads_spread || !plan.heads_nb) return false;
+  if ((int)d_u2_dual.size() != conf.SharedLayers || !d_ep_init_h2) return false;
+  if (!d_w3_init || Kp % 128 != 0 || (size_t)B * Hp * Wp * Fp * sizeof(float) >= ((size_t)1 << 32)) return false;
+  const H2Tower t = wino_h2_tower(B);
+  return t.chained && t.ns == 2 && t.chunk * 2 == B;
+}
+
+int agz_net::forward_half_reserve(int B) {
+  const H2Tower t = wino_h2_tower(B);
+  int r = wino_h2_reserve(B, t, nullptr);
+  if (r != AGZ_OK) return r;
+  const size_t need = (size_t)B * (3 * HW + conf.ActionSpace + conf.FC);
+  if (need > hs_cap) {
+    AGZ_HIP_TRY(hipStreamSynchronize(ctx->stream));
+    if (d_hs) hipFree(d_hs);
+    d_hs = nullptr; hs_cap = 0;
+    AGZ_HIP_TRY(hipMalloc(&d_hs, need * sizeof(float)));
+    hs_cap = need;
+  }
+  return AGZ_OK;
+}
+
+int agz_net::forward_half(int B, int half, hipStream_t st, float* policy_dev, float* value_dev, hipEvent_t mid) {
+  const int nb = B / 2, b0 = half * nb;
+  const FwdPlan plan = fwd_plan(B);
+  const H2Tower t = wino_h2_tower(B);
+  ConvArgs a{};
+  a.M = nb * HW; a.HW = HW; a.W = W; a.Wp = Wp; a.HpWp = Hp * Wp;
+  a.x = d_act_in + (size_t)b0 * Hp * Wp * Fp; a.w = d_w_init; a.ep = d_ep_init_h2; a.y = d_actA + (size_t)b0 * Hp * Wp * Kp;
+  a.Cin_p = Fp; a.Cout_p = Kp; a.Ntot = Kp;
+  a.n_ntiles = ceil_div(a.Ntot, 128); a.n_mtiles = ceil_div(a.M, 128);
+  a.splits = 1; a.per = 0; a.ws = nullptr; a.raw = 0;
+  AGZ_HIP_TRY(hipMemsetAsync(d_amax + b0, 0, (size_t)nb * sizeof(unsigned), st));
+  a.amax_out = d_amax + b0;
+  hipLaunchKernelGGL((conv3x3_x3_kernel<false>), dim3(a.n_mtiles * a.n_ntiles), dim3(256), 0, st, a, d_w3_init);
+  const int L = conf.SharedLayers;
+  for (int l = 0; l < L; l++) {
+    wino_h2c_block(l, B, b0, half, t, st, d_actA, d_actB);
+    if (mid && l == L / 2) AGZ_HIP_TRY(hipEventRecord(mid, st));
+  }
+  HeadArgs h{};
+  h.x = d_actB; h.conv = d_head_conv; h.bn = d_head_bn; h.Wp = d_Wp; h.bp = d_bp; h.W1 = d_W1; h.b1 = d_b1; h.W2 = d_W2;
+  h.b2 = d_b2; h.policy = policy_dev; h.value = value_dev;
+  h.H = H; h.W = W; h.HW = HW; h.Wp_ = Wp; h.HpWp = Hp * Wp; h.Kp = Kp; h.A = conf.ActionSpace; h.FC = conf.FC;
+  heads_spread_range(h, plan.heads_nb, B, b0, nb, st);
+  AGZ_HIP_TRY(hipGetLastError());
+  return AGZ_OK;
+}
+
 int agz_net::forward_packed(int B, float* policy_dev, float* value_dev) {
   AGZ_REQUIRE(committed, AGZ_E_STATE, "agz_net: infer before agz_net_commit");
   AGZ_REQUIRE(B >= 1 && B <= max_batch, AGZ_E_INVALID, "agz_net: batch %d exceeds allocated %d", B, max_batch);
@@ -1126,89 +1269,31 @@
   bool tower_done = false;
   if (!tower_done && wino_h2_ok) {
     AGZ_REQUIRE((int)d_u2_dual.size() == conf.SharedLayers, AGZ_E_STATE, "agz_net: Winograd fp16x2 weights not built");
-    const int npos = (wino_tm + 2) * (wino_tm + 2);
-    const int tpb = ceil_div(H, wino_tm) * ceil_div(W, wino_tm);
     const bool wide = plan.wino_wide;
-    static const int chunk_env = [] { const char* e = getenv("AGZ_WINO_H2_CHUNK"); return e ? atoi(e) : 0; }();
-    static const int queues_env = [] { const char* e = getenv("AGZ_WINO_H2_QUEUES"); return e ? atoi(e) : 0; }();
-    const int queues_want = queues_env > 0 ? queues_env : (tower_queues > 0 ? tower_queues : (B >= 256 ? 2 : 1));
-    const int chunk_max = (int)std::min<size_t>((size_t)B, ((((size_t)1 << 32) - 1) / ((size_t)npos * Kp * 4) - 127) / tpb);
-    int chunk = chunk_env >= 1 ? std::min(chunk_env, chunk_max) : chunk_max;
-    const int ns = (queues_want == 2 && B >= 64) ? 2 : 1;
-    if (ns == 2 && chunk >= B) chunk = (B + 1) / 2;
-    const size_t v_elems = wino_h2_rows(npos, (size_t)chunk * tpb) * Kp, m_elems = 2 * v_elems;
-    static const int form_env = [] { const char* e = getenv("AGZ_WINO_H2_FORM"); return e ? atoi(e) : -1; }();
-    const int form_want = wino_form >= 0 ? wino_form : form_env;
-    const bool chained = form_want != 0 && (int)d_u2c_dual.size() == conf.SharedLayers && agz::wino_h2c_ok(H, W, wino_tm, Kp);
-    const int n_scr = chained ? ceil_div(B, chunk) : ns;
-    if (v_elems * n_scr > wino_v_cap) {
-      AGZ_HIP_TRY(hipStreamSynchronize(ctx->stream));
-      if (ctx->stream2) AGZ_HIP_TRY(hipStreamSynchronize(ctx->stream2));
-      if (d_wV) hipFree(d_wV);
-      if (d_wM) hipFree(d_wM);
-      d_wV = d_wM = nullptr; wino_chunk_cap = 0;
-      AGZ_HIP_TRY(hipMalloc(&d_wV, v_elems * n_scr * sizeof(float)));
-      AGZ_HIP_TRY(hipMalloc(&d_wM, m_elems * n_scr * sizeof(float)));
-      wino_v_cap = v_elems * n_scr; wino_chunk_cap = 0;
-    }
-    const size_t wm_board = chained ? (size_t)tpb * (Kp >> 5) * 2 : (size_t)tpb * (Kp >> 6);
-    const size_t need_amax = (size_t)(conf.SharedLayers + 1) * B + wm_board * B;
-    if (need_amax > amax_cap) {
-      AGZ_HIP_TRY(hipStreamSynchronize(ctx->stream));
-      if (ctx->stream2) AGZ_HIP_TRY(hipStreamSynchronize(ctx->stream2));
-      if (d_amax) hipFree(d_amax);
-      d_amax = nullptr; amax_cap = 0;
-      AGZ_HIP_TRY(hipMalloc(&d_amax, need_amax * sizeof(unsigned)));
-      amax_cap = need_amax;
-      amax0_done = false;
+    const H2Tower tw = wino_h2_tower(B);
+    const int chunk = tw.chunk, ns = tw.ns;
+    const size_t v_elems = tw.v_elems, m_elems = tw.m_elems, wm_board = tw.wm_board;
+    const bool chained = tw.chained;
+    {
+      bool amax_moved = false;
+      const int rr = wino_h2_reserve(B, tw, &amax_moved);
+      if (rr != AGZ_OK) return rr;
+      if (amax_moved) amax0_done = false;
     }
     float* d_wave_max = reinterpret_cast<float*>(d_amax + (size_t)(conf.SharedLayers + 1) * B);
     if (!amax0_done)
       hipLaunchKernelGGL(board_amax_kernel, dim3(B), dim3(256), 0, ctx->stream, cur, d_amax, HW, W, Wp, Hp * Wp, Kp, (const float*)nullptr);
     if (ns == 2) {
-      if (!ctx->stream2) {
-        AGZ_HIP_TRY(hipStreamCreateWithFlags(&ctx->stream2, hipStreamNonBlocking));
-        AGZ_HIP_TRY(hipEventCreateWithFlags(&ctx->ev_fork, hipEventDisableTiming));
-        AGZ_HIP_TRY(hipEventCreateWithFlags(&ctx->ev_join, hipEventDisableTiming));
-      }
+      { const int rs = ctx->ensure_stream2(); if (rs != AGZ_OK) return rs; }
       AGZ_HIP_TRY(hipEventRecord(ctx->ev_fork, ctx->stream));
       AGZ_HIP_TRY(hipStreamWaitEvent(ctx->stream2, ctx->ev_fork, 0));
     }
     for (int l = 0; chained && l < conf.SharedLayers; l++) {
       ProfScope ps(ctx, AGZ_PROF_CONV);
       int ci = 0;
-      const size_t wmb = (size_t)tpb * (Kp >> 5);
       const bool last = l + 1 == conf.SharedLayers;
-      for (int b0 = 0; b0 < B; b0 += chunk, ci++) {
-        const int q = ci % ns;
-        hipStream_t st = q ? ctx->stream2 : ctx->stream;
-        WinoH2Args hh{};
-        WinoArgs& wa = hh.w;
-        wa.x = cur + (size_t)b0 * Hp * Wp * Kp; wa.y = nxt + (size_t)b0 * Hp * Wp * Kp;
-        wa.V = d_wV + (size_t)ci * v_elems; wa.Mb = d_wM + (size_t)ci * m_elems; wa.ep = d_ep_h2[l];
-        wa.B = std::min(chunk, B - b0); wa.H = H; wa.W = W; wa.Hp = Hp; wa.Wp = Wp; wa.C = Kp; wa.Cout_p = Kp; wa.Ntot = 2 * Kp;
-        hh.U2c = d_u2c_dual[l]; hh.w_unscale = 1.f; hh.tm = wino_tm;
-        hh.amax_in = d_amax + (size_t)l * B + b0;
-        hh.amax_next = last ? nullptr : d_amax + (size_t)(l + 1) * B + b0;
-        hh.amax_true = l == 0 ? reinterpret_cast<const float*>(d_amax + b0) : nullptr;
-        hh.wm_prev = d_wave_max + ((size_t)((l + 1) & 1) * B + b0) * wmb;
-        hh.wm_out = d_wave_max + ((size_t)(l & 1) * B + b0) * wmb;
-        hh.g1 = wino_g1[l]; hh.g0 = wino_g0[l];
-        {
-          static const int gemm_env = [] {
-            const char* e = getenv("AGZ_WINO_H2_GEMM");
-            const int v = e ? atoi(e) : 0;
-            if (v == 0 || (((v & 63) == 1 || (v & 63) == 2) && (v >> 6) <= 1)) return v;
-            fprintf(stderr, "libagz: AGZ_WINO_H2_GEMM=%s ignored (want 1 or 2, optionally + 64)\n", e);
-            return 0;
-          }();
-          const int gv = wino_gemm > 0 ? wino_gemm : gemm_env;
-          hh.gemm_variant = gv & 63; hh.temporal_stores = (gv >> 6) & 1;
-        }
-        if (l == 0) agz::wino_h2c_in(ctx, hh, st);
-        agz::wino_h2c_gemm(ctx, hh, st);
-        agz::wino_h2c_oi(ctx, hh, last, st, form_want == 1 ? 1 : 4);
-      }
+      for (int b0 = 0; b0 < B; b0 += chunk, ci++)
+        wino_h2c_block(l, B, b0, ci, tw, (ci % ns) ? ctx->stream2 : (hipStream_t)ctx->stream, cur, nxt);
       if (last) std::swap(cur, nxt);
     }
     for (int l = 0; !chained && l < conf.SharedLayers; l++) {
@@ -1326,13 +1411,7 @@
         AGZ_HIP_TRY(hipMalloc(&d_hs, need * sizeof(float)));
         hs_cap = need;
       }
-      h.feat = d_hs; h.cols = d_hs + (size_t)B * 3 * HW;
-      hipLaunchKernelGGL(heads_feat_kernel, dim3(ceil_div(HW, 4), B), dim3(256), 0, ctx->stream, h);
-      if (plan.heads_nb)
-        hipLaunchKernelGGL(heads_fc_nb_kernel<4>, dim3(ceil_div(conf.ActionSpace + conf.FC, 64), ceil_div(B, 4)), dim3(1024), 0, ctx->stream, h, B);
-      else
-        hipLaunchKernelGGL(heads_fc_kernel, dim3(ceil_div(conf.ActionSpace + conf.FC, 64), B), dim3(1024), 0, ctx->stream, h);
-      hipLaunchKernelGGL(heads_out_kernel, dim3(B), dim3(256), 0, ctx->stream, h);
+      heads_spread_range(h, plan.heads_nb, B, 0, B, ctx->stream);
     } else {
       hipLaunchKernelGGL(heads_kernel, dim3(B), dim3(256), smem, ctx->stream, h);
     }
diff --git a/agogo_amd/csrc/net.hpp b/agogo_amd/csrc/net.hpp
--- a/agogo_amd/csrc/net.hpp
+++ b/agogo_amd/csrc/net.hpp
@@ -34,6 +34,7 @@
                         const unsigned* ranges = nullptr, const RawWeights* pre = nullptr);
 bool conv3x3_raw_wino_h2_fits(int B, int H, int W, int Cin_p, int Cout_p);
 void wino_raw_scratch_free(WinoRawScratch* sc);
+struct HeadArgs;
 }
 
 struct agz_net {
@@ -116,4 +117,12 @@
   struct FwdPlan { bool half_init, half_dual, small, forced_split, latency, heads_spread, split_ok, heads_nb, wino_wide; };
   FwdPlan fwd_plan(int B) const;
   int min_same_batch(int n, int G) const;
+  struct H2Tower { int npos, tpb, chunk, ns, n_scr, form_want; bool chained; size_t v_elems, m_elems, wm_board; };
+  H2Tower wino_h2_tower(int B) const;
+  int wino_h2_reserve(int B, const H2Tower& t, bool* amax_moved);
+  void wino_h2c_block(int l, int B, int b0, int ci, const H2Tower& t, hipStream_t st, float* cur, float* nxt);
+  void heads_spread_range(agz::HeadArgs h, bool nb4, int B, int b0, int nb, hipStream_t st);
+  bool half_ok(int B) const;
+  int forward_half_reserve(int B);
+  int forward_half(int B, int half, hipStream_t st, float* policy_dev, float* value_dev, hipEvent_t mid);
 };
diff --git a/include/agz_debug.h b/include/agz_debug.h
--- a/include/agz_debug.h
+++ b/include/agz_debug.h
@@ -34,6 +34,9 @@
 int agz_arena_set_prep_compact(agz_arena* arena, int on);
 int agz_arena_last_prep_batch(agz_arena* arena, int* boards, int* roots);
 
+int agz_arena_set_split(agz_arena* arena, int mode);
+int agz_arena_split_steps(agz_arena* arena, int64_t* split, int64_t* joined, int* last_split);
+
 int agz_trainer_set_dma_forward(agz_trainer* t, int on);
 
 int agz_net_min_same_batch(agz_net* net, int n, int G, int* batch);
```

After: 43160 (median of 6 runs). 1.02x the previous value.
